# stcodeer/Frequency-wised_All-in-One_Image_Restoration_Model

Measured on AMD Instinct MI355X. Metric: training images/sec @128x128, higher is better.
Workload: dtype bf16; 1 GPU; BASELINE configs[1]: Uformer encoder+decoder (all_3_bands, L=3, freq MSA), denoise sigma=25, 128x128, phase-2 train step (fwd+bwd+Adam, DropPath on); per_gpu_batch=16, global_batch=16, parallelism=dp1, hip_graph=True

## Files before the change

### frequency-wised_all-in-one_image_restoration_model_amd/csrc/fw_gemm.hip

```cpp
#include "fw_common.h"
#include <stdio.h>
#include <string.h>
#include <stdlib.h>

namespace {
static thread_local char g_last_kernel[96] = "";
template <typename T> constexpr const char* tname() { return sizeof(T) == 2 ? "bf16" : "float"; }
#define FW_B(x) ((x) ? "true" : "false")
#define FW_KNAME(...) snprintf(g_last_kernel, sizeof g_last_kernel, __VA_ARGS__)

struct GemmArgs {
    const char* X; const char* W; char* C;
    long ldx, ldw, ldc;
    int M, N, K;
    int x_op, w_op;
    const float* bias;
    int act; float slope;
    const char* aux; long ldaux;
    const float* rowscale; int rows_per_scale;
    const float* residual; long ldr;
    int out_f32;
    int accumulate;
    int splitk; int kper;
    char* C2; long ldc2;
    float* xsum;
    long c_zstride, xsum_zstride;
    float alpha;
    int staged;
    int dbg;
};

constexpr int LDS_ROW = 128;
FW_DEV int swz(int row) { return ((row ^ (row >> 3)) & 7) << 4; }
constexpr int BM = 128;

FW_DEV unsigned xcd_contiguous(unsigned lin, unsigned total) {
    const unsigned xcd = lin & 7, q = total >> 3, r = total & 7;
    return (xcd < r ? xcd * (q + 1) : r * (q + 1) + (xcd - r) * q) + (lin >> 3);
}

template <typename T> FW_DEV uint4 apply_gelu16(const uint4& v) {
    float f[TT<T>::E16];
    unpack16<T>(v, f);
#pragma unroll
    for (int i = 0; i < TT<T>::E16; ++i) f[i] = gelu_t<T>(f[i]);
    return pack16<T>(f);
}

template <typename T>
FW_DEV void epi_fetch(const GemmArgs& a, uint4& ext, int mc, int nc, int z) {
    if (a.act == 2) {
        const T* ap = reinterpret_cast<const T*>(a.aux) + (long)mc * a.ldaux + nc;
        if (sizeof(T) == 4) ext = *reinterpret_cast<const uint4*>(ap);
        else { const uint2 t = *reinterpret_cast<const uint2*>(ap); ext.x = t.x; ext.y = t.y; }
    } else if (a.residual && z == 0) {
        ext = *reinterpret_cast<const uint4*>(a.residual + (long)mc * a.ldr + nc);
    }
}
FW_DEV f32x4 epi_bias(const GemmArgs& a, int nc, int z) {
    return (a.bias && z == 0) ? *reinterpret_cast<const f32x4*>(a.bias + nc) : f32x4{0.f, 0.f, 0.f, 0.f};
}
template <typename T>
FW_DEV void epi_apply(const GemmArgs& a, const f32x4& bias, const uint4& ext, const f32x4& acc, int m, int n0, float rs, int z) {
    float v[4];
#pragma unroll
    for (int r = 0; r < 4; ++r) v[r] = acc[r] * a.alpha + bias[r];
    if (a.act == 1) {
#pragma unroll
        for (int r = 0; r < 4; ++r) v[r] = lrelu_f(v[r], a.slope);
    } else if (a.act == 2) {
        float x[4];
        if (sizeof(T) == 4) { x[0] = __uint_as_float(ext.x); x[1] = __uint_as_float(ext.y); x[2] = __uint_as_float(ext.z); x[3] = __uint_as_float(ext.w); }
        else { x[0] = __uint_as_float(ext.x << 16); x[1] = __uint_as_float(ext.x & 0xffff0000u);
               x[2] = __uint_as_float(ext.y << 16); x[3] = __uint_as_float(ext.y & 0xffff0000u); }
#pragma unroll
        for (int r = 0; r < 4; ++r) v[r] *= gelu_grad_t<T>(x[r]);
    } else if (a.act == 3) {
#pragma unroll
        for (int r = 0; r < 4; ++r) v[r] = gelu_t<T>(v[r]);
    }
    if (a.rowscale) {
#pragma unroll
        for (int r = 0; r < 4; ++r) v[r] *= rs;
    }
    if (a.residual && z == 0) {
        uint4 rr = ext;
        if (a.act == 2) rr = *reinterpret_cast<const uint4*>(a.residual + (long)m * a.ldr + n0);
        v[0] += __uint_as_float(rr.x); v[1] += __uint_as_float(rr.y); v[2] += __uint_as_float(rr.z); v[3] += __uint_as_float(rr.w);
    }
    if (a.C2) {
        T* c2 = reinterpret_cast<T*>(a.C2) + (long)m * a.ldc2 + n0;
        const float g0 = gelu_t<T>(v[0]), g1 = gelu_t<T>(v[1]), g2 = gelu_t<T>(v[2]), g3 = gelu_t<T>(v[3]);
        if (sizeof(T) == 4) *reinterpret_cast<f32x4*>(c2) = f32x4{g0, g1, g2, g3};
        else *reinterpret_cast<uint2*>(c2) = make_uint2(pack_bf2(g0, g1), pack_bf2(g2, g3));
    }
    if (a.out_f32) {
        float* cp = reinterpret_cast<float*>(a.C) + (long)z * a.c_zstride + (long)m * a.ldc + n0;
        if (a.accumulate && a.c_zstride == 0) {
            if (a.accumulate == 1 && a.splitk == 1) {
                const f32x4 old = *reinterpret_cast<const f32x4*>(cp);
                *reinterpret_cast<f32x4*>(cp) = f32x4{old[0] + v[0], old[1] + v[1], old[2] + v[2], old[3] + v[3]};
            } else {
#pragma unroll
                for (int r = 0; r < 4; ++r) atomicAdd(cp + r, v[r]);
            }
        } else {
            *reinterpret_cast<f32x4*>(cp) = f32x4{v[0], v[1], v[2], v[3]};
        }
    } else {
        T* cp = reinterpret_cast<T*>(a.C) + (long)m * a.ldc + n0;
        if (sizeof(T) == 4) *reinterpret_cast<f32x4*>(cp) = f32x4{v[0], v[1], v[2], v[3]};
        else *reinterpret_cast<uint2*>(cp) = make_uint2(pack_bf2(v[0], v[1]), pack_bf2(v[2], v[3]));
    }
}

template <typename T, int ROWS>
struct StageDirect {
    static constexpr int NL = ROWS / 32;
    uint4 r[NL];
    FW_MEM void load(const char* base, long ld, int row0, int rows_total, int kbyte0, int kbytes_end, int op) {
        const int tid = threadIdx.x;
#pragma unroll
        for (int t = 0; t < NL; ++t) {
            const int cid = tid + 256 * t;
            const int row = cid >> 3, kb = kbyte0 + (cid & 7) * 16;
            const int rr = row0 + row < rows_total ? row0 + row : rows_total - 1;
            r[t] = *reinterpret_cast<const uint4*>(base + (long)rr * ld * TT<T>::SZ + (kb < kbytes_end ? kb : 0));
        }
#pragma unroll
        for (int t = 0; t < NL; ++t) {
            const int cid = tid + 256 * t;
            const int row = cid >> 3, kb = kbyte0 + (cid & 7) * 16;
            uint4 v = r[t];
            if (op == 1) v = apply_gelu16<T>(v);
            const int valid = row0 + row < rows_total ? kbytes_end - kb : 0;
            v.x = valid > 0 ? v.x : 0u; v.y = valid > 4 ? v.y : 0u; v.z = valid > 8 ? v.z : 0u; v.w = valid > 12 ? v.w : 0u;
            r[t] = v;
        }
    }
    FW_MEM void store(char* tile) const {
        const int tid = threadIdx.x;
#pragma unroll
        for (int t = 0; t < NL; ++t) {
            const int cid = tid + 256 * t;
            const int row = cid >> 3;
            *reinterpret_cast<uint4*>(tile + row * LDS_ROW + (((cid & 7) * 16) ^ swz(row))) = r[t];
        }
    }
};

template <typename T, int ROWS>
struct StageTrans {
    static constexpr int E = TT<T>::E16;
    static constexpr int IB = ROWS / E;
    static constexpr int KT = 128 / TT<T>::SZ;
    static constexpr int NTHR = IB * (KT / 4);
    uint4 r[4];
    FW_MEM void load(const char* base, long ld, int row0, int rows_total, int k0, int k_end, int op) {
        const int tid = threadIdx.x;
        const int ib = tid % IB, kb = tid / IB;
#pragma unroll
        for (int kk = 0; kk < 4; ++kk) {
            const int k = k0 + kb * 4 + kk;
            uint4 v = make_uint4(0, 0, 0, 0);
            if (tid < NTHR && k < k_end && row0 + ib * E < rows_total) {
                v = *reinterpret_cast<const uint4*>(base + ((long)k * ld + row0 + ib * E) * TT<T>::SZ);
                if (op == 1) v = apply_gelu16<T>(v);
            }
            r[kk] = v;
        }
    }
    FW_MEM void accum(float (&s)[TT<T>::E16]) const {
#pragma unroll
        for (int kk = 0; kk < 4; ++kk) {
            float f[TT<T>::E16];
            unpack16<T>(r[kk], f);
#pragma unroll
            for (int e = 0; e < TT<T>::E16; ++e) s[e] += f[e];
        }
    }
    FW_MEM void store(char* tile) const {
        const int tid = threadIdx.x;
        if (tid >= NTHR) return;
        const int ib = tid % IB, kb = tid / IB;
        if constexpr (sizeof(T) == 4) {
            const int r0 = ib * 4, cb = kb * 16;
            *reinterpret_cast<uint4*>(tile + (r0 + 0) * LDS_ROW + (cb ^ swz(r0 + 0))) = make_uint4(r[0].x, r[1].x, r[2].x, r[3].x);
            *reinterpret_cast<uint4*>(tile + (r0 + 1) * LDS_ROW + (cb ^ swz(r0 + 1))) = make_uint4(r[0].y, r[1].y, r[2].y, r[3].y);
            *reinterpret_cast<uint4*>(tile + (r0 + 2) * LDS_ROW + (cb ^ swz(r0 + 2))) = make_uint4(r[0].z, r[1].z, r[2].z, r[3].z);
            *reinterpret_cast<uint4*>(tile + (r0 + 3) * LDS_ROW + (cb ^ swz(r0 + 3))) = make_uint4(r[0].w, r[1].w, r[2].w, r[3].w);
        } else {
            const int r0 = ib * 8, cb = kb * 8;
            const unsigned w0[4] = {r[0].x, r[0].y, r[0].z, r[0].w};
            const unsigned w1[4] = {r[1].x, r[1].y, r[1].z, r[1].w};
            const unsigned w2[4] = {r[2].x, r[2].y, r[2].z, r[2].w};
            const unsigned w3[4] = {r[3].x, r[3].y, r[3].z, r[3].w};
#pragma unroll
            for (int d = 0; d < 4; ++d) {
                uint2 lo = make_uint2(__builtin_amdgcn_perm(w1[d], w0[d], 0x05040100u),
                                      __builtin_amdgcn_perm(w3[d], w2[d], 0x05040100u));
                uint2 hi = make_uint2(__builtin_amdgcn_perm(w1[d], w0[d], 0x07060302u),
                                      __builtin_amdgcn_perm(w3[d], w2[d], 0x07060302u));
                *reinterpret_cast<uint2*>(tile + (r0 + 2 * d) * LDS_ROW + (cb ^ swz(r0 + 2 * d))) = lo;
                *reinterpret_cast<uint2*>(tile + (r0 + 2 * d + 1) * LDS_ROW + (cb ^ swz(r0 + 2 * d + 1))) = hi;
            }
        }
    }
};

typedef __attribute__((address_space(3))) void lds_void_t;
typedef __attribute__((address_space(1))) const void glb_void_t;
template <typename T, int ROWS>
FW_DEV void glds_issue(const char* base, long ld, int row0, int rows_total, int kbyte0, char* tile) {
    const int lane = threadIdx.x & 63, wave = threadIdx.x >> 6;
#pragma unroll
    for (int it = 0; it < ROWS / 32; ++it) {
        const int R0 = (wave * (ROWS / 32) + it) * 8;
        const int r = R0 + (lane >> 3), p = lane & 7;
        int gr = row0 + r;
        if (gr >= rows_total) gr = rows_total - 1;
        const char* g = base + (long)gr * ld * TT<T>::SZ + kbyte0 + ((p ^ (swz(r) >> 4)) << 4);
        __builtin_amdgcn_global_load_lds((glb_void_t*)g, (lds_void_t*)(tile + R0 * LDS_ROW), 16, 0, 0);
    }
}

template <typename T, int ROWS> struct StageDirectAcc : StageDirect<T, ROWS> {
    FW_MEM void accum(float (&)[TT<T>::E16]) const {}
};
template <typename T, int ROWS, bool TRANS> struct Stage;
template <typename T, int ROWS> struct Stage<T, ROWS, false> : StageDirectAcc<T, ROWS> {
    FW_MEM void fetch(const char* base, long ld, int row0, int rows_total, int k0, int k_end, int op) {
        this->load(base, ld, row0, rows_total, k0 * TT<T>::SZ, k_end * TT<T>::SZ, op);
    }
};
template <typename T, int ROWS> struct Stage<T, ROWS, true> : StageTrans<T, ROWS> {
    FW_MEM void fetch(const char* base, long ld, int row0, int rows_total, int k0, int k_end, int op) {
        this->load(base, ld, row0, rows_total, k0, k_end, op);
    }
};

FW_DEV uint4 frag_sw(const char* tile, int row0, int chunk) {
    const int l = lane_id();
    const int row = row0 + (l & 15);
    return *reinterpret_cast<const uint4*>(tile + row * LDS_ROW + ((chunk * 64 + ((l >> 4) << 4)) ^ swz(row)));
}

template <typename T, int BN, bool XT, bool WT, bool GX, bool GW>
__global__ __launch_bounds__(256) void gemm_kernel(GemmArgs a) {
    constexpr int KT = 128 / TT<T>::SZ;
    constexpr int WM = (BN == 128) ? 4 : 2;
    constexpr int XBYTES = BM * LDS_ROW, WBYTES = BN * LDS_ROW;
    extern __shared__ __attribute__((aligned(16))) char smem[];
    auto xs = [&](int i) -> char* { return smem + i * (XBYTES + WBYTES); };
    auto ws = [&](int i) -> char* { return smem + i * (XBYTES + WBYTES) + XBYTES; };

    const int wave = threadIdx.x >> 6;
    int bx = blockIdx.x, by = blockIdx.y, bz = blockIdx.z;
    {
        const unsigned total = gridDim.x * gridDim.y * gridDim.z;
        if (gridDim.z > 1) {
            const unsigned lin = blockIdx.x + gridDim.x * (blockIdx.y + gridDim.y * blockIdx.z);
            const unsigned w = xcd_contiguous(lin, total);
            bx = (int)(w % gridDim.x);
            by = (int)((w / gridDim.x) % gridDim.y);
            bz = (int)(w / (gridDim.x * gridDim.y));
        } else if (gridDim.z == 1 && gridDim.y > 1) {
            const unsigned lin = blockIdx.x + gridDim.x * blockIdx.y;
            const unsigned w = xcd_contiguous(lin, total);
            const unsigned per_band = 8 * gridDim.y;
            const unsigned band = w / per_band, first = band * 8;
            const unsigned gsz = min(gridDim.x - first, 8u);
            bx = (int)(first + (w % per_band) % gsz);
            by = (int)((w % per_band) / gsz);
        }
    }
    const int m_blk = bx * BM, n_blk = by * BN;
    const int wm0 = (BN == 128) ? (wave & 1) * 64 : wave * 32;
    const int wn0 = (BN == 128) ? (wave >> 1) * 64 : 0;

    const int k_begin = bz * a.kper;
    const int k_end = min(a.K, k_begin + a.kper);
    const int nsteps = (k_end - k_begin + KT - 1) / KT;

    f32x4 acc[4][WM];
    zero_acc(acc);

    Stage<T, BM, XT> sx;
    Stage<T, BN, WT> sw;
    float xsum[TT<T>::E16];
#pragma unroll
    for (int e = 0; e < TT<T>::E16; ++e) xsum[e] = 0.f;
    const bool do_xsum = XT && a.xsum != nullptr && by == 0;
    if (nsteps > 0) {
        if constexpr (GX) glds_issue<T, BM>(a.X, a.ldx, m_blk, a.M, k_begin * TT<T>::SZ, xs(0));
        else { sx.fetch(a.X, a.ldx, m_blk, a.M, k_begin, k_end, a.x_op); if (do_xsum) sx.accum(xsum); }
        if constexpr (GW) glds_issue<T, BN>(a.W, a.ldw, n_blk, a.N, k_begin * TT<T>::SZ, ws(0));
        else sw.fetch(a.W, a.ldw, n_blk, a.N, k_begin, k_end, a.w_op);
        if constexpr (!GX) sx.store(xs(0));
        if constexpr (!GW) sw.store(ws(0));
    }
    __syncthreads();
    for (int s = 0; s < nsteps; ++s) {
        const int cur = s & 1;
        if (s + 1 < nsteps) {
            if constexpr (GX) glds_issue<T, BM>(a.X, a.ldx, m_blk, a.M, (k_begin + (s + 1) * KT) * TT<T>::SZ, xs(cur ^ 1));
            else { sx.fetch(a.X, a.ldx, m_blk, a.M, k_begin + (s + 1) * KT, k_end, a.x_op); if (do_xsum) sx.accum(xsum); }
            if constexpr (GW) glds_issue<T, BN>(a.W, a.ldw, n_blk, a.N, (k_begin + (s + 1) * KT) * TT<T>::SZ, ws(cur ^ 1));
            else sw.fetch(a.W, a.ldw, n_blk, a.N, k_begin + (s + 1) * KT, k_end, a.w_op);
        }
#pragma unroll
        for (int c = 0; c < 2; ++c) {
            uint4 af[4], bfr[WM];
#pragma unroll
            for (int m = 0; m < 4; ++m) af[m] = frag_sw(ws(cur), wn0 + 16 * m, c);
#pragma unroll
            for (int n = 0; n < WM; ++n) bfr[n] = frag_sw(xs(cur), wm0 + 16 * n, c);
#pragma unroll
            for (int m = 0; m < 4; ++m)
#pragma unroll
                for (int n = 0; n < WM; ++n) mma_chunk<T>(acc[m][n], af[m], bfr[n]);
        }
        if (s + 1 < nsteps) {
            if constexpr (!GX) sx.store(xs(cur ^ 1));
            if constexpr (!GW) sw.store(ws(cur ^ 1));
        }
        __syncthreads();
    }

    if constexpr (XT) {
        if (a.xsum != nullptr && by == 0) {
            constexpr int E = TT<T>::E16, IB = BM / E;
            float* red = reinterpret_cast<float*>(smem);
            if (threadIdx.x < BM) red[threadIdx.x] = 0.f;
            __syncthreads();
            if ((int)threadIdx.x < IB * ((128 / TT<T>::SZ) / 4)) {
                const int ib = threadIdx.x % IB;
#pragma unroll
                for (int e = 0; e < E; ++e) atomicAdd(&red[ib * E + e], xsum[e]);
            }
            __syncthreads();
            if (threadIdx.x < BM && m_blk + (int)threadIdx.x < a.M) {
                if (a.xsum_zstride > 0) a.xsum[(long)bz * a.xsum_zstride + m_blk + threadIdx.x] = red[threadIdx.x];
                else atomicAdd(a.xsum + m_blk + threadIdx.x, red[threadIdx.x]);
            }
        }
    }
    const int l = lane_id();
    f32x4 bias4[4];
#pragma unroll
    for (int nt = 0; nt < 4; ++nt) {
        const int n0 = n_blk + wn0 + nt * 16 + ((l >> 4) << 2);
        bias4[nt] = epi_bias(a, n0 < a.N ? n0 : 0, bz);
    }
#pragma unroll
    for (int mt = 0; mt < WM; ++mt) {
        const int m = m_blk + wm0 + mt * 16 + (l & 15);
        const int mc = m < a.M ? m : a.M - 1;
        const float rs = a.rowscale ? a.rowscale[mc / a.rows_per_scale] : 1.0f;
        uint4 ext[4];
#pragma unroll
        for (int nt = 0; nt < 4; ++nt) {
            const int n0 = n_blk + wn0 + nt * 16 + ((l >> 4) << 2);
            epi_fetch<T>(a, ext[nt], mc, n0 < a.N ? n0 : 0, bz);
        }
#pragma unroll
        for (int nt = 0; nt < 4; ++nt) {
            const int n0 = n_blk + wn0 + nt * 16 + ((l >> 4) << 2);
            if (m < a.M && n0 < a.N) epi_apply<T>(a, bias4[nt], ext[nt], acc[nt][mt], m, n0, rs, bz);
        }
    }
}

FW_DEV int swz256(int r) { return ((r & 3) << 2) | ((r >> 2) & 3); }

FW_DEV uint4 frag_tr256(const char* tile, int m0, int chunk) {
    const int l = lane_id();
    const int r = chunk * 32 + ((l >> 4) << 3) + ((l >> 2) & 3);
    const int ch = (m0 >> 3) + ((l & 3) >> 1), sub = (l & 1) << 3;
    const char* p0 = tile + 256 * r + ((ch ^ swz256(r)) << 4) + sub;
    const char* p1 = tile + 256 * (r + 4) + ((ch ^ swz256(r + 4)) << 4) + sub;
    const uint2 lo = __builtin_bit_cast(uint2, __builtin_amdgcn_ds_read_tr16_b64_v4i16((fw_lds_s16x4*)p0));
    const uint2 hi = __builtin_bit_cast(uint2, __builtin_amdgcn_ds_read_tr16_b64_v4i16((fw_lds_s16x4*)p1));
    return make_uint4(lo.x, lo.y, hi.x, hi.y);
}

template <typename T, int WM, bool PLAIN>
FW_DEV void tile_epilogue(const GemmArgs& a, const f32x4 (&acc)[4][WM], int m_blk, int n_blk, int wm0, int wn0, int bz) {
    const int l = lane_id();
    f32x4 bias4[4];
#pragma unroll
    for (int nt = 0; nt < 4; ++nt) {
        const int n0 = n_blk + wn0 + nt * 16 + ((l >> 4) << 2);
        bias4[nt] = epi_bias(a, n0 < a.N ? n0 : 0, bz);
    }
    if constexpr (PLAIN) {
#pragma unroll
        for (int mt = 0; mt < WM; ++mt) {
            const int m = m_blk + wm0 + mt * 16 + (l & 15);
            if (m >= a.M) continue;
            if (a.out_f32) {
                float* cp = reinterpret_cast<float*>(a.C) + (long)bz * a.c_zstride + (long)m * a.ldc;
#pragma unroll
                for (int nt = 0; nt < 4; ++nt) {
                    const int n0 = n_blk + wn0 + nt * 16 + ((l >> 4) << 2);
                    if (n0 < a.N) *reinterpret_cast<f32x4*>(cp + n0) = acc[nt][mt] + bias4[nt];
                }
            } else {
                T* cp = reinterpret_cast<T*>(a.C) + (long)m * a.ldc;
#pragma unroll
                for (int nt = 0; nt < 4; ++nt) {
                    const int n0 = n_blk + wn0 + nt * 16 + ((l >> 4) << 2);
                    if (n0 < a.N) {
                        const f32x4 v = acc[nt][mt] + bias4[nt];
                        if (sizeof(T) == 4) *reinterpret_cast<f32x4*>(cp + n0) = v;
                        else *reinterpret_cast<uint2*>(cp + n0) = make_uint2(pack_bf2(v[0], v[1]), pack_bf2(v[2], v[3]));
                    }
                }
            }
        }
    } else {
        const bool tw = sizeof(T) == 2 && a.alpha == 1.0f && !a.out_f32 && !a.rowscale && !a.residual && !a.accumulate;
        if (tw && a.act == 2 && !a.C2) {
            auto fetchA = [&](uint2 (&ext)[4], int mt) {
                const int m = m_blk + wm0 + mt * 16 + (l & 15);
                const T* ap = reinterpret_cast<const T*>(a.aux) + (long)(m < a.M ? m : a.M - 1) * a.ldaux;
#pragma unroll
                for (int nt = 0; nt < 4; ++nt) {
                    const int n0 = n_blk + wn0 + nt * 16 + ((l >> 4) << 2);
                    ext[nt] = *reinterpret_cast<const uint2*>(ap + (n0 < a.N ? n0 : 0));
                }
            };
            auto applyA = [&](const uint2 (&ext)[4], int mt) {
                const int m = m_blk + wm0 + mt * 16 + (l & 15);
                if (m >= a.M) return;
                T* cp = reinterpret_cast<T*>(a.C) + (long)m * a.ldc;
#pragma unroll
                for (int nt = 0; nt < 4; ++nt) {
                    const int n0 = n_blk + wn0 + nt * 16 + ((l >> 4) << 2);
                    if (n0 >= a.N) continue;
                    const f32x4 v = acc[nt][mt] + bias4[nt];
                    const float x0 = __uint_as_float(ext[nt].x << 16), x1 = __uint_as_float(ext[nt].x & 0xffff0000u);
                    const float x2 = __uint_as_float(ext[nt].y << 16), x3 = __uint_as_float(ext[nt].y & 0xffff0000u);
                    *reinterpret_cast<uint2*>(cp + n0) = make_uint2(pack_bf2(v[0] * gelu_grad_poly(x0), v[1] * gelu_grad_poly(x1)),
                                                                    pack_bf2(v[2] * gelu_grad_poly(x2), v[3] * gelu_grad_poly(x3)));
                }
            };
            uint2 ea[4], eb[4];
            fetchA(ea, 0);
#pragma unroll
            for (int mt = 0; mt < WM; mt += 2) {
                if (mt + 1 < WM) fetchA(eb, mt + 1);
                applyA(ea, mt);
                if (mt + 1 < WM) {
                    if (mt + 2 < WM) fetchA(ea, mt + 2);
                    applyA(eb, mt + 1);
                }
            }
            return;
        }
        if (tw && a.act == 0 && a.C2) {
#pragma unroll
            for (int mt = 0; mt < WM; ++mt) {
                const int m = m_blk + wm0 + mt * 16 + (l & 15);
                if (m >= a.M) continue;
                T* cp = reinterpret_cast<T*>(a.C) + (long)m * a.ldc;
                T* c2 = reinterpret_cast<T*>(a.C2) + (long)m * a.ldc2;
#pragma unroll
                for (int nt = 0; nt < 4; ++nt) {
                    const int n0 = n_blk + wn0 + nt * 16 + ((l >> 4) << 2);
                    if (n0 >= a.N) continue;
                    const f32x4 v = acc[nt][mt] + bias4[nt];
                    *reinterpret_cast<uint2*>(cp + n0) = make_uint2(pack_bf2(v[0], v[1]), pack_bf2(v[2], v[3]));
                    *reinterpret_cast<uint2*>(c2 + n0) = make_uint2(pack_bf2(gelu_poly(v[0]), gelu_poly(v[1])), pack_bf2(gelu_poly(v[2]), gelu_poly(v[3])));
                }
            }
            return;
        }
        if (a.act == 0 && a.residual && a.out_f32 && !a.C2 && a.alpha == 1.0f && !a.accumulate && a.splitk == 1 && a.c_zstride == 0) {
            auto fetchC = [&](f32x4 (&ext)[4], int mt) {
                const int m = m_blk + wm0 + mt * 16 + (l & 15);
                const float* rp = a.residual + (long)(m < a.M ? m : a.M - 1) * a.ldr;
#pragma unroll
                for (int nt = 0; nt < 4; ++nt) {
                    const int n0 = n_blk + wn0 + nt * 16 + ((l >> 4) << 2);
                    ext[nt] = *reinterpret_cast<const f32x4*>(rp + (n0 < a.N ? n0 : 0));
                }
            };
            auto applyC = [&](const f32x4 (&ext)[4], int mt) {
                const int m = m_blk + wm0 + mt * 16 + (l & 15);
                if (m >= a.M) return;
                const float rs = a.rowscale ? a.rowscale[m / a.rows_per_scale] : 1.0f;
                float* cp = reinterpret_cast<float*>(a.C) + (long)m * a.ldc;
#pragma unroll
                for (int nt = 0; nt < 4; ++nt) {
                    const int n0 = n_blk + wn0 + nt * 16 + ((l >> 4) << 2);
                    if (n0 < a.N) *reinterpret_cast<f32x4*>(cp + n0) = (acc[nt][mt] + bias4[nt]) * rs + ext[nt];
                }
            };
            f32x4 ea[4], eb[4];
            fetchC(ea, 0);
#pragma unroll
            for (int mt = 0; mt < WM; mt += 2) {
                if (mt + 1 < WM) fetchC(eb, mt + 1);
                applyC(ea, mt);
                if (mt + 1 < WM) {
                    if (mt + 2 < WM) fetchC(ea, mt + 2);
                    applyC(eb, mt + 1);
                }
            }
            return;
        }
        auto fetch = [&](uint4 (&ext)[4], int mt) {
            const int m = m_blk + wm0 + mt * 16 + (l & 15);
            const int mc = m < a.M ? m : a.M - 1;
#pragma unroll
            for (int nt = 0; nt < 4; ++nt) {
                const int n0 = n_blk + wn0 + nt * 16 + ((l >> 4) << 2);
                epi_fetch<T>(a, ext[nt], mc, n0 < a.N ? n0 : 0, bz);
            }
        };
        auto apply = [&](const uint4 (&ext)[4], int mt) {
            const int m = m_blk + wm0 + mt * 16 + (l & 15);
            const int mc = m < a.M ? m : a.M - 1;
            const float rs = a.rowscale ? a.rowscale[mc / a.rows_per_scale] : 1.0f;
#pragma unroll
            for (int nt = 0; nt < 4; ++nt) {
                const int n0 = n_blk + wn0 + nt * 16 + ((l >> 4) << 2);
                if (m < a.M && n0 < a.N) epi_apply<T>(a, bias4[nt], ext[nt], acc[nt][mt], m, n0, rs, bz);
            }
        };
        uint4 ea[4], eb[4];
        fetch(ea, 0);
#pragma unroll
        for (int mt = 0; mt < WM; mt += 2) {
            if (mt + 1 < WM) fetch(eb, mt + 1);
            apply(ea, mt);
            if (mt + 1 < WM) {
                if (mt + 2 < WM) fetch(ea, mt + 2);
                apply(eb, mt + 1);
            }
        }
    }
}
static inline bool plain_epilogue(const GemmArgs& a) {
    return a.act == 0 && !a.rowscale && !a.residual && !a.C2 && a.alpha == 1.0f && !(a.accumulate && a.c_zstride == 0);
}

template <int N> FW_DEV void wait_vmcnt() { asm volatile("s_waitcnt vmcnt(%0)" ::"n"(N) : "memory"); }
FW_DEV void glds16_asm(const char* gsrc, char* lds_dst) {
    unsigned keep;
    const unsigned dst = __builtin_amdgcn_readfirstlane((unsigned)(uintptr_t)(lds_void_t*)lds_dst);
    asm volatile("s_mov_b32 %0, m0\n\ts_mov_b32 m0, %2\n\ts_nop 0\n\tglobal_load_lds_dwordx4 %1, off\n\ts_mov_b32 m0, %0"
                 : "=&s"(keep) : "v"(gsrc), "s"(dst) : "memory");
}

template <int KT> struct GldsKm {
    static constexpr int NI = KT / 16;
    const char* src[NI];
    long kstride;
    int loff[NI];
    FW_MEM void init(const char* base, long ld, int col0, int cols_total, int k0) {
        const int lane = threadIdx.x & 63, wave = threadIdx.x >> 6;
        kstride = ld * 2;
#pragma unroll
        for (int it = 0; it < NI; ++it) {
            const int R0 = wave * (KT / 4) + it * 4;
            const int r = R0 + (lane >> 4), p = lane & 15;
            int col = col0 + ((p ^ swz256(r)) << 3);
            if (col >= cols_total) col = 0;
            src[it] = base + ((long)(k0 + r) * ld + col) * 2;
            loff[it] = R0 * 256;
        }
    }
    FW_MEM void issue(int step, char* tile) const {
        const long off = (long)step * KT * kstride;
#pragma unroll
        for (int it = 0; it < NI; ++it) glds16_asm(src[it] + off, tile + loff[it]);
    }
};
template <typename T, int ROWS> struct GldsKc {
    static constexpr int NI = ROWS / 32;
    const char* src[NI];
    int loff[NI];
    FW_MEM void init(const char* base, long ld, int row0, int rows_total, int kbyte0) {
        const int lane = threadIdx.x & 63, wave = threadIdx.x >> 6;
#pragma unroll
        for (int it = 0; it < NI; ++it) {
            const int R0 = (wave * NI + it) * 8;
            const int r = R0 + (lane >> 3), p = lane & 7;
            int gr = row0 + r;
            if (gr >= rows_total) gr = rows_total - 1;
            src[it] = base + (long)gr * ld * TT<T>::SZ + kbyte0 + ((p ^ (swz(r) >> 4)) << 4);
            loff[it] = R0 * LDS_ROW;
        }
    }
    FW_MEM void issue(int step, char* tile) const {
#pragma unroll
        for (int it = 0; it < NI; ++it) glds16_asm(src[it] + (long)step * 128, tile + loff[it]);
    }
};

constexpr int ROW64 = 64;
FW_DEV int swz64(int r) { return (r >> 2) & 3; }
template <typename T, int ROWS> struct GldsKc64 {
    static constexpr int NI = ROWS / 64;
    const char* src[NI];
    int loff[NI];
    FW_MEM void init(const char* base, long ld, int row0, int rows_total, int kbyte0) {
        const int lane = threadIdx.x & 63, wave = threadIdx.x >> 6;
#pragma unroll
        for (int it = 0; it < NI; ++it) {
            const int R0 = (wave * NI + it) * 16;
            const int r = R0 + (lane >> 2), p = lane & 3;
            int gr = row0 + r;
            if (gr >= rows_total) gr = rows_total - 1;
            src[it] = base + (long)gr * ld * TT<T>::SZ + kbyte0 + ((p ^ swz64(r)) << 4);
            loff[it] = R0 * ROW64;
        }
    }
    FW_MEM void issue(int step, char* tile) const {
#pragma unroll
        for (int it = 0; it < NI; ++it) glds16_asm(src[it] + (long)step * ROW64, tile + loff[it]);
    }
};
FW_DEV uint4 frag_sw64(const char* tile, int row0) {
    const int l = lane_id();
    const int row = row0 + (l & 15);
    return *reinterpret_cast<const uint4*>(tile + row * ROW64 + (((l >> 4) ^ swz64(row)) << 4));
}

constexpr int EPI_LD = 136;
template <int WM>
FW_DEV void tile_epilogue_staged(const GemmArgs& a, const f32x4 (&acc)[4][WM], int m_blk, int n_blk, int wm0, int wn0, char* stage, int mode) {
    const int l = lane_id();
    char* mine = stage + (threadIdx.x >> 6) * (16 * WM * EPI_LD);
    f32x4 bias4[4];
#pragma unroll
    for (int nt = 0; nt < 4; ++nt) {
        const int n0 = n_blk + wn0 + nt * 16 + ((l >> 4) << 2);
        bias4[nt] = epi_bias(a, n0 < a.N ? n0 : 0, 0);
    }
    const int rsub = l >> 3, cb = (l & 7) * 16;
    const int ncol = n_blk + wn0 + (l & 7) * 8;
    const bool col_ok = ncol < a.N;
    auto rows_out = [&](char* C, long ldc) {
#pragma unroll
        for (int it = 0; it < 2 * WM; ++it) {
            const int r = it * 8 + rsub, m = m_blk + wm0 + r;
            const uint4 v = *reinterpret_cast<const uint4*>(mine + r * EPI_LD + cb);
            if (m < a.M && col_ok) *reinterpret_cast<uint4*>(C + ((long)m * ldc + ncol) * 2) = v;
        }
    };
    if (mode == 2) {
#pragma unroll
        for (int it = 0; it < 2 * WM; ++it) {
            const int r = it * 8 + rsub, m = m_blk + wm0 + r;
            const long mc = m < a.M ? m : a.M - 1;
            const uint4 v = *reinterpret_cast<const uint4*>(a.aux + (mc * a.ldaux + (col_ok ? ncol : 0)) * 2);
            *reinterpret_cast<uint4*>(mine + r * EPI_LD + cb) = v;
        }
        __builtin_amdgcn_fence(__ATOMIC_RELEASE, "wavefront");
        asm volatile("s_waitcnt vmcnt(0) lgkmcnt(0)" ::: "memory");
        __builtin_amdgcn_fence(__ATOMIC_ACQUIRE, "wavefront");
    }
#pragma unroll
    for (int pass = 0; pass < 2; ++pass) {
        if (pass == 1 && mode != 1) break;
#pragma unroll
        for (int mt = 0; mt < WM; ++mt) {
            char* rowp = mine + (mt * 16 + (l & 15)) * EPI_LD + ((l >> 4) << 3);
#pragma unroll
            for (int nt = 0; nt < 4; ++nt) {
                f32x4 v = acc[nt][mt] + bias4[nt];
                if (mode == 2) {
                    const uint2 e = *reinterpret_cast<const uint2*>(rowp + nt * 32);
                    v[0] *= gelu_grad_poly(__uint_as_float(e.x << 16)); v[1] *= gelu_grad_poly(__uint_as_float(e.x & 0xffff0000u));
                    v[2] *= gelu_grad_poly(__uint_as_float(e.y << 16)); v[3] *= gelu_grad_poly(__uint_as_float(e.y & 0xffff0000u));
                } else if (pass == 1) {
                    v[0] = gelu_poly(v[0]); v[1] = gelu_poly(v[1]); v[2] = gelu_poly(v[2]); v[3] = gelu_poly(v[3]);
                }
                *reinterpret_cast<uint2*>(rowp + nt * 32) = make_uint2(pack_bf2(v[0], v[1]), pack_bf2(v[2], v[3]));
            }
        }
        __builtin_amdgcn_fence(__ATOMIC_RELEASE, "wavefront");
        asm volatile("s_waitcnt lgkmcnt(0)" ::: "memory");
        __builtin_amdgcn_fence(__ATOMIC_ACQUIRE, "wavefront");
        if (pass == 0) rows_out(a.C, a.ldc); else rows_out(a.C2, a.ldc2);
        if (pass == 0 && mode == 1) {
            __builtin_amdgcn_fence(__ATOMIC_RELEASE, "wavefront");
            asm volatile("s_waitcnt lgkmcnt(0)" ::: "memory");
            __builtin_amdgcn_fence(__ATOMIC_ACQUIRE, "wavefront");
        }
    }
}
static inline int staged_mode(const GemmArgs& a) {
    if (a.out_f32 || a.alpha != 1.0f || a.rowscale || a.residual || a.accumulate || a.c_zstride || a.splitk != 1 || a.N % 8 || a.ldc % 8) return -1;
    if (((uintptr_t)a.C & 15)) return -1;
    if (a.act == 0 && !a.C2) return 0;
    if (a.act == 0 && a.C2) return (a.ldc2 % 8 || ((uintptr_t)a.C2 & 15)) ? -1 : 1;
    if (a.act == 2 && !a.C2) return (a.ldaux % 8 || ((uintptr_t)a.aux & 15)) ? -1 : 2;
    return -1;
}

template <bool XT, int KT, int NS, bool PLAIN>
FW_DEV void tr_ring_tile(const GemmArgs& a, int bx, int by, int bz, char* smem) {
    using T = bf16raw;
    static_assert(NS == 2 || NS == 3, "ring depth");
    constexpr int WM = 4;
    constexpr bool X64 = !XT && KT == 32;
    constexpr int XB = XT ? KT * 256 : 128 * (X64 ? ROW64 : LDS_ROW), WB = KT * 256, STAGE = XB + WB;
    constexpr int LPS = (XT ? KT / 16 : (X64 ? 2 : 4)) + KT / 16;
    auto xs = [&](int i) -> char* { return smem + i * STAGE; };
    auto ws = [&](int i) -> char* { return smem + i * STAGE + XB; };
    const int wave = threadIdx.x >> 6;
    const int m_blk = bx * 128, n_blk = by * 128;
    const int wm0 = (wave & 1) * 64, wn0 = (wave >> 1) * 64;
    const int k_begin = bz * a.kper;
    const int k_end = min(a.K, k_begin + a.kper);
    const int nsteps = (k_end - k_begin) / KT;

    f32x4 acc[4][WM], xsacc[WM];
    zero_acc(acc);
#pragma unroll
    for (int m = 0; m < WM; ++m) xsacc[m] = f32x4{0.f, 0.f, 0.f, 0.f};
    const bool do_xsum = XT && a.xsum != nullptr && by == 0 && wn0 == 0;
    const uint4 ones = make_uint4(0x3F803F80u, 0x3F803F80u, 0x3F803F80u, 0x3F803F80u);

    GldsKm<KT> gw;
    gw.init(a.W, a.ldw, n_blk, a.N, k_begin);
    GldsKm<XT ? KT : 16> gxm;
    GldsKc<T, BM> gxc;
    GldsKc64<T, BM> gxc64;
    if constexpr (XT) gxm.init(a.X, a.ldx, m_blk, a.M, k_begin);
    else if constexpr (X64) gxc64.init(a.X, a.ldx, m_blk, a.M, k_begin * 2);
    else gxc.init(a.X, a.ldx, m_blk, a.M, k_begin * 2);
    auto issue = [&](int step, int buf) {
        if constexpr (XT) gxm.issue(step, xs(buf));
        else if constexpr (X64) gxc64.issue(step, xs(buf));
        else gxc.issue(step, xs(buf));
        gw.issue(step, ws(buf));
    };
#pragma unroll
    for (int p = 0; p < NS - 1; ++p)
        if (p < nsteps) issue(p, p);
    int buf = 0;
    for (int s = 0; s < nsteps; ++s) {
        const int younger = min(NS - 2, nsteps - 1 - s);
        if (younger >= NS - 2) wait_vmcnt<(NS - 2) * LPS>();
        else wait_vmcnt<0>();
        __builtin_amdgcn_s_barrier();
        asm volatile("" ::: "memory");
        if (s + NS - 1 < nsteps) issue(s + NS - 1, buf == 0 ? NS - 1 : buf - 1);
#pragma unroll
        for (int c = 0; c < KT / 32; ++c) {
            uint4 af[4], bfr[WM];
#pragma unroll
            for (int m = 0; m < 4; ++m) af[m] = frag_tr256(ws(buf), wn0 + 16 * m, c);
#pragma unroll
            for (int n = 0; n < WM; ++n) bfr[n] = XT ? frag_tr256(xs(buf), wm0 + 16 * n, c) : (X64 ? frag_sw64(xs(buf), wm0 + 16 * n) : frag_sw(xs(buf), wm0 + 16 * n, c));
#pragma unroll
            for (int m = 0; m < 4; ++m)
#pragma unroll
                for (int n = 0; n < WM; ++n) mma_chunk<T>(acc[m][n], af[m], bfr[n]);
            if (do_xsum) {
#pragma unroll
                for (int n = 0; n < WM; ++n) mma_chunk<T>(xsacc[n], ones, bfr[n]);
            }
        }
        buf = buf + 1 == NS ? 0 : buf + 1;
    }
    const int l = lane_id();
    if (do_xsum && (l >> 4) == 0) {
#pragma unroll
        for (int n = 0; n < WM; ++n) {
            const int m = m_blk + wm0 + n * 16 + l;
            if (m < a.M) {
                if (a.xsum_zstride > 0) a.xsum[(long)bz * a.xsum_zstride + m] = xsacc[n][0];
                else atomicAdd(a.xsum + m, xsacc[n][0]);
            }
        }
    }
    if (a.staged >= 0 && (size_t)NS * STAGE >= (size_t)4 * 16 * WM * EPI_LD) {
        __syncthreads();
        tile_epilogue_staged<WM>(a, acc, m_blk, n_blk, wm0, wn0, smem, a.staged);
        return;
    }
    tile_epilogue<T, WM, PLAIN>(a, acc, m_blk, n_blk, wm0, wn0, bz);
}

template <bool XT, int KT, int NS, bool PLAIN>
__global__ __launch_bounds__(256, KT == 32 ? 3 : 2) void gemm_tr_ring_kernel(GemmArgs a) {
    extern __shared__ __attribute__((aligned(16))) char smem[];
    int bx = blockIdx.x, by = blockIdx.y, bz = blockIdx.z;
    {
        const unsigned total = gridDim.x * gridDim.y * gridDim.z;
        if (gridDim.z > 1) {
            const unsigned lin = blockIdx.x + gridDim.x * (blockIdx.y + gridDim.y * blockIdx.z);
            const unsigned w = xcd_contiguous(lin, total);
            bx = (int)(w % gridDim.x);
            by = (int)((w / gridDim.x) % gridDim.y);
            bz = (int)(w / (gridDim.x * gridDim.y));
        } else if (gridDim.z == 1 && gridDim.y > 1) {
            const unsigned lin = blockIdx.x + gridDim.x * blockIdx.y;
            const unsigned w = xcd_contiguous(lin, total);
            const unsigned per_band = 8 * gridDim.y;
            const unsigned band = w / per_band, first = band * 8;
            const unsigned gsz = min(gridDim.x - first, 8u);
            bx = (int)(first + (w % per_band) % gsz);
            by = (int)((w % per_band) / gsz);
        }
    }
    tr_ring_tile<XT, KT, NS, PLAIN>(a, bx, by, bz, smem);
}

__global__ __launch_bounds__(256, 3) void gemm_wgrad_group_kernel(const GemmArgs* __restrict__ probs, const int4* __restrict__ items) {
    extern __shared__ __attribute__((aligned(16))) char smem[];
    const int4 it = items[blockIdx.x];
    if (it.x < 0) return;
    const GemmArgs a = probs[it.x];
    if (a.c_zstride > 0) tr_ring_tile<true, 32, 3, true>(a, it.y, it.z, it.w, smem);
    else tr_ring_tile<true, 32, 3, false>(a, it.y, it.z, it.w, smem);
}

template <bool PLAIN>
FW_DEV void tr_big_tile(const GemmArgs& a, int bx, int by, int bz, char* smem) {
    using T = bf16raw;
    constexpr int KT = 32, NS = 3, WM = 8, IMG = KT * 256, STAGE = 4 * IMG, LPS = 4;
    const int lane = threadIdx.x & 63, wave = threadIdx.x >> 6;
    const int m_blk = bx * 256, n_blk = by * 256;
    const int wm0 = (wave & 1) * 128, wn0 = (wave >> 1) * 64;
    const int k_begin = bz * a.kper;
    const int k_end = min(a.K, k_begin + a.kper);
    const int nsteps = (k_end - k_begin) / KT;
    const char* src[4]; int off[4];
    {
        const bool isw = wave >= 4;
        const int half = (wave >> 1) & 1, rg = wave & 1;
        const char* base = isw ? a.W : a.X;
        const long ld = isw ? a.ldw : a.ldx;
        const int col0 = (isw ? n_blk : m_blk) + half * 128, cols = isw ? a.N : a.M;
#pragma unroll
        for (int it = 0; it < 4; ++it) {
            const int R0 = rg * 16 + it * 4, r = R0 + (lane >> 4), p = lane & 15;
            int col = col0 + ((p ^ swz256(r)) << 3);
            if (col >= cols) col = 0;
            src[it] = base + ((long)(k_begin + r) * ld + col) * 2;
            off[it] = (isw ? 2 * IMG : 0) + half * IMG + R0 * 256;
        }
    }
    const long kstride = (wave >= 4 ? a.ldw : a.ldx) * 2;
    auto issue = [&](int step, int buf) {
        char* st = smem + buf * STAGE;
#pragma unroll
        for (int it = 0; it < 4; ++it) glds16_asm(src[it] + (long)step * KT * kstride, st + off[it]);
    };
    f32x4 acc[4][WM];
    zero_acc(acc);
    float xs[WM];
#pragma unroll
    for (int m = 0; m < WM; ++m) xs[m] = 0.f;
    const bool do_xsum = a.xsum != nullptr && by == 0 && wn0 == 0;
    typedef __attribute__((ext_vector_type(2))) __bf16 bf2_t;
    const bf2_t ones2 = __builtin_bit_cast(bf2_t, 0x3F803F80u);
#pragma unroll
    for (int p = 0; p < NS - 1; ++p)
        if (p < nsteps) issue(p, p);
    int buf = 0;
    for (int s = 0; s < nsteps; ++s) {
        const int younger = min(NS - 2, nsteps - 1 - s);
        if (younger >= NS - 2) wait_vmcnt<(NS - 2) * LPS>();
        else wait_vmcnt<0>();
        __builtin_amdgcn_s_barrier();
        asm volatile("" ::: "memory");
        if (s + NS - 1 < nsteps) issue(s + NS - 1, buf == 0 ? NS - 1 : buf - 1);
        const char* st = smem + buf * STAGE;
        uint4 af[4], bfr[WM];
#pragma unroll
        for (int m = 0; m < 4; ++m) af[m] = frag_tr256(st + 2 * IMG + (wn0 >> 7) * IMG, (wn0 & 127) + 16 * m, 0);
#pragma unroll
        for (int n = 0; n < WM; ++n) bfr[n] = frag_tr256(st + (wm0 >> 7) * IMG, 16 * n, 0);
#pragma unroll
        for (int m = 0; m < 4; ++m)
#pragma unroll
            for (int n = 0; n < WM; ++n) mma_chunk<T>(acc[m][n], af[m], bfr[n]);
        if (do_xsum) {
#pragma unroll
            for (int n = 0; n < WM; ++n) {
                xs[n] = __builtin_amdgcn_fdot2_f32_bf16(__builtin_bit_cast(bf2_t, bfr[n].x), ones2, xs[n], false);
                xs[n] = __builtin_amdgcn_fdot2_f32_bf16(__builtin_bit_cast(bf2_t, bfr[n].y), ones2, xs[n], false);
                xs[n] = __builtin_amdgcn_fdot2_f32_bf16(__builtin_bit_cast(bf2_t, bfr[n].z), ones2, xs[n], false);
                xs[n] = __builtin_amdgcn_fdot2_f32_bf16(__builtin_bit_cast(bf2_t, bfr[n].w), ones2, xs[n], false);
            }
        }
        buf = buf + 1 == NS ? 0 : buf + 1;
    }
    const int l = lane_id();
    if (do_xsum) {
#pragma unroll
        for (int n = 0; n < WM; ++n) {
            float v = xs[n];
            v += __shfl_xor(v, 16, 64); v += __shfl_xor(v, 32, 64);
            const int m = m_blk + wm0 + n * 16 + l;
            if ((l >> 4) == 0 && m < a.M) {
                if (a.xsum_zstride > 0) a.xsum[(long)bz * a.xsum_zstride + m] = v;
                else atomicAdd(a.xsum + m, v);
            }
        }
    }
    tile_epilogue<T, WM, PLAIN>(a, acc, m_blk, n_blk, wm0, wn0, bz);
}
__global__ __launch_bounds__(512) void gemm_wgrad_group_big_kernel(const GemmArgs* __restrict__ probs, const int4* __restrict__ items) {
    extern __shared__ __attribute__((aligned(16))) char smem[];
    const int4 it = items[blockIdx.x];
    if (it.x < 0) return;
    const GemmArgs a = probs[it.x];
    if (a.c_zstride > 0) tr_big_tile<true>(a, it.y, it.z, it.w, smem);
    else tr_big_tile<false>(a, it.y, it.z, it.w, smem);
}

template <bool XT, int KT, int NS, bool PLAIN>
int launch_tr_ring_p(const GemmArgs& a, hipStream_t st) {
    const size_t lds = (size_t)NS * ((XT ? KT * 256 : 128 * ((KT == 32) ? ROW64 : LDS_ROW)) + KT * 256);
    FW_SET_LDS_ONCE((gemm_tr_ring_kernel<XT, KT, NS, PLAIN>), lds);
    FW_KNAME("gemm_tr_ring_kernel<%s,%d,%d,%s>", FW_B(XT), KT, NS, FW_B(PLAIN));
    hipLaunchKernelGGL((gemm_tr_ring_kernel<XT, KT, NS, PLAIN>), dim3(fw_cdiv(a.M, 128), fw_cdiv(a.N, 128), a.splitk), dim3(256), lds, st, a);
    FW_LAUNCH_RET();
}
template <bool XT, int KT, int NS>
int launch_tr_ring(const GemmArgs& a, hipStream_t st) {
    return plain_epilogue(a) ? launch_tr_ring_p<XT, KT, NS, true>(a, st) : launch_tr_ring_p<XT, KT, NS, false>(a, st);
}

template <typename T, int BN, int NS, bool PLAIN>
__global__ __launch_bounds__(256) void gemm_ring_kernel(GemmArgs a) {
    constexpr int KT = 128 / TT<T>::SZ;
    constexpr int WM = (BN == 128) ? 4 : 2;
    constexpr int XBYTES = BM * LDS_ROW, WBYTES = BN * LDS_ROW, STAGE = XBYTES + WBYTES;
    constexpr int LPS = BM / 32 + BN / 32;
    extern __shared__ __attribute__((aligned(16))) char smem[];
    auto xs = [&](int i) -> char* { return smem + i * STAGE; };
    auto ws = [&](int i) -> char* { return smem + i * STAGE + XBYTES; };
    const int wave = threadIdx.x >> 6;
    int bx = blockIdx.x, by = blockIdx.y, bz = blockIdx.z;
    {
        const unsigned total = gridDim.x * gridDim.y * gridDim.z;
        if (gridDim.z > 1) {
            const unsigned lin = blockIdx.x + gridDim.x * (blockIdx.y + gridDim.y * blockIdx.z);
            const unsigned w = xcd_contiguous(lin, total);
            bx = (int)(w % gridDim.x);
            by = (int)((w / gridDim.x) % gridDim.y);
            bz = (int)(w / (gridDim.x * gridDim.y));
        } else if (gridDim.z == 1 && gridDim.y > 1) {
            const unsigned lin = blockIdx.x + gridDim.x * blockIdx.y;
            const unsigned w = xcd_contiguous(lin, total);
            const unsigned per_band = 8 * gridDim.y;
            const unsigned band = w / per_band, first = band * 8;
            const unsigned gsz = min(gridDim.x - first, 8u);
            bx = (int)(first + (w % per_band) % gsz);
            by = (int)((w % per_band) / gsz);
        }
    }
    const int m_blk = bx * BM, n_blk = by * BN;
    const int wm0 = (BN == 128) ? (wave & 1) * 64 : wave * 32;
    const int wn0 = (BN == 128) ? (wave >> 1) * 64 : 0;
    const int k_begin = bz * a.kper;
    const int k_end = min(a.K, k_begin + a.kper);
    const int nsteps = (k_end - k_begin) / KT;

    f32x4 acc[4][WM];
    zero_acc(acc);
    GldsKc<T, BM> gx;
    GldsKc<T, BN> gw;
    gx.init(a.X, a.ldx, m_blk, a.M, k_begin * TT<T>::SZ);
    gw.init(a.W, a.ldw, n_blk, a.N, k_begin * TT<T>::SZ);
    auto issue = [&](int step, int buf) {
        gx.issue(step, xs(buf));
        gw.issue(step, ws(buf));
    };
#pragma unroll
    for (int p = 0; p < NS - 1; ++p)
        if (p < nsteps) issue(p, p);
    int buf = 0;
    for (int s = 0; s < nsteps; ++s) {
        const int younger = min(NS - 2, nsteps - 1 - s);
        if (younger >= NS - 2) wait_vmcnt<(NS - 2) * LPS>();
        else wait_vmcnt<0>();
        __builtin_amdgcn_s_barrier();
        asm volatile("" ::: "memory");
        if (s + NS - 1 < nsteps) issue(s + NS - 1, buf == 0 ? NS - 1 : buf - 1);
#pragma unroll
        for (int c = 0; c < 2; ++c) {
            uint4 af[4], bfr[WM];
#pragma unroll
            for (int m = 0; m < 4; ++m) af[m] = frag_sw(ws(buf), wn0 + 16 * m, c);
#pragma unroll
            for (int n = 0; n < WM; ++n) bfr[n] = frag_sw(xs(buf), wm0 + 16 * n, c);
#pragma unroll
            for (int m = 0; m < 4; ++m)
#pragma unroll
                for (int n = 0; n < WM; ++n) mma_chunk<T>(acc[m][n], af[m], bfr[n]);
        }
        buf = buf + 1 == NS ? 0 : buf + 1;
    }
    if constexpr (sizeof(T) == 2) {
        if (a.staged >= 0 && (size_t)NS * STAGE >= (size_t)4 * 16 * WM * EPI_LD) {
            __syncthreads();
            tile_epilogue_staged<WM>(a, acc, m_blk, n_blk, wm0, wn0, smem, a.staged);
            return;
        }
    }
    tile_epilogue<T, WM, PLAIN>(a, acc, m_blk, n_blk, wm0, wn0, bz);
}

template <typename T, int BN, int NS, bool PLAIN>
int launch_ring_p(const GemmArgs& a, hipStream_t st) {
    const size_t lds = (size_t)NS * (BM + BN) * LDS_ROW;
    FW_SET_LDS_ONCE((gemm_ring_kernel<T, BN, NS, PLAIN>), lds);
    dim3 grid(fw_cdiv(a.M, BM), fw_cdiv(a.N, BN), a.splitk);
    FW_KNAME("gemm_ring_kernel<%s,%d,%d,%s>", tname<T>(), BN, NS, FW_B(PLAIN));
    hipLaunchKernelGGL((gemm_ring_kernel<T, BN, NS, PLAIN>), grid, dim3(256), lds, st, a);
    FW_LAUNCH_RET();
}
template <typename T, int BN, int NS>
int launch_ring(const GemmArgs& a, hipStream_t st) {
    return plain_epilogue(a) ? launch_ring_p<T, BN, NS, true>(a, st) : launch_ring_p<T, BN, NS, false>(a, st);
}

template <typename T, int BN, int NS, bool PLAIN>
__global__ __launch_bounds__(256) void gemm_ring64_kernel(GemmArgs a) {
    constexpr int KT = ROW64 / TT<T>::SZ;
    constexpr int WM = (BN == 128) ? 4 : 2;
    constexpr int XBYTES = BM * ROW64, WBYTES = BN * ROW64, STAGE = XBYTES + WBYTES;
    constexpr int LPS = BM / 64 + BN / 64;
    static_assert(NS >= 3, "ring depth");
    extern __shared__ __attribute__((aligned(16))) char smem[];
    auto xs = [&](int i) -> char* { return smem + i * STAGE; };
    auto ws = [&](int i) -> char* { return smem + i * STAGE + XBYTES; };
    const int wave = threadIdx.x >> 6;
    int bx = blockIdx.x, by = blockIdx.y, bz = blockIdx.z;
    {
        const unsigned total = gridDim.x * gridDim.y * gridDim.z;
        if (gridDim.z > 1) {
            const unsigned lin = blockIdx.x + gridDim.x * (blockIdx.y + gridDim.y * blockIdx.z);
            const unsigned w = xcd_contiguous(lin, total);
            bx = (int)(w % gridDim.x);
            by = (int)((w / gridDim.x) % gridDim.y);
            bz = (int)(w / (gridDim.x * gridDim.y));
        } else if (gridDim.z == 1 && gridDim.y > 1) {
            const unsigned lin = blockIdx.x + gridDim.x * blockIdx.y;
            const unsigned w = xcd_contiguous(lin, total);
            const unsigned per_band = 8 * gridDim.y;
            const unsigned band = w / per_band, first = band * 8;
            const unsigned gsz = min(gridDim.x - first, 8u);
            bx = (int)(first + (w % per_band) % gsz);
            by = (int)((w % per_band) / gsz);
        }
    }
    const int m_blk = bx * BM, n_blk = by * BN;
    const int wm0 = (BN == 128) ? (wave & 1) * 64 : wave * 32;
    const int wn0 = (BN == 128) ? (wave >> 1) * 64 : 0;
    const int k_begin = bz * a.kper;
    const int k_end = min(a.K, k_begin + a.kper);
    const int nsteps = (k_end - k_begin) / KT;

    f32x4 acc[4][WM];
    zero_acc(acc);
    GldsKc64<T, BM> gx;
    GldsKc64<T, BN> gw;
    gx.init(a.X, a.ldx, m_blk, a.M, k_begin * TT<T>::SZ);
    gw.init(a.W, a.ldw, n_blk, a.N, k_begin * TT<T>::SZ);
    auto issue = [&](int step, int buf) {
        gx.issue(step, xs(buf));
        gw.issue(step, ws(buf));
    };
#pragma unroll
    for (int p = 0; p < NS - 1; ++p)
        if (p < nsteps) issue(p, p);
    int buf = 0;
    for (int s = 0; s < nsteps; ++s) {
        const int younger = min(NS - 2, nsteps - 1 - s);
        if (younger >= NS - 2) wait_vmcnt<(NS - 2) * LPS>();
        else if (younger == NS - 3) wait_vmcnt<(NS - 3) * LPS>();
        else wait_vmcnt<0>();
        __builtin_amdgcn_s_barrier();
        asm volatile("" ::: "memory");
        if (s + NS - 1 < nsteps) issue(s + NS - 1, buf == 0 ? NS - 1 : buf - 1);
        uint4 af[4], bfr[WM];
#pragma unroll
        for (int m = 0; m < 4; ++m) af[m] = frag_sw64(ws(buf), wn0 + 16 * m);
#pragma unroll
        for (int n = 0; n < WM; ++n) bfr[n] = frag_sw64(xs(buf), wm0 + 16 * n);
#pragma unroll
        for (int m = 0; m < 4; ++m)
#pragma unroll
            for (int n = 0; n < WM; ++n) mma_chunk<T>(acc[m][n], af[m], bfr[n]);
        buf = buf + 1 == NS ? 0 : buf + 1;
    }
    if constexpr (sizeof(T) == 2) {
        if (a.staged >= 0 && (size_t)NS * STAGE >= (size_t)4 * 16 * WM * EPI_LD) {
            __syncthreads();
            tile_epilogue_staged<WM>(a, acc, m_blk, n_blk, wm0, wn0, smem, a.staged);
            return;
        }
    }
    tile_epilogue<T, WM, PLAIN>(a, acc, m_blk, n_blk, wm0, wn0, bz);
}

template <typename T, int BN, int NS, bool PLAIN>
int launch_ring64_p(const GemmArgs& a, hipStream_t st) {
    const size_t lds = (size_t)NS * (BM + BN) * ROW64;
    FW_SET_LDS_ONCE((gemm_ring64_kernel<T, BN, NS, PLAIN>), lds);
    dim3 grid(fw_cdiv(a.M, BM), fw_cdiv(a.N, BN), a.splitk);
    FW_KNAME("gemm_ring64_kernel<%s,%d,%d,%s>", tname<T>(), BN, NS, FW_B(PLAIN));
    hipLaunchKernelGGL((gemm_ring64_kernel<T, BN, NS, PLAIN>), grid, dim3(256), lds, st, a);
    FW_LAUNCH_RET();
}
template <typename T, int BN, int NS>
int launch_ring64(const GemmArgs& a, hipStream_t st) {
    return plain_epilogue(a) ? launch_ring64_p<T, BN, NS, true>(a, st) : launch_ring64_p<T, BN, NS, false>(a, st);
}

template <bool WT, bool PLAIN>
__global__ __launch_bounds__(512) void gemm_big_kernel(GemmArgs a) {
    using T = bf16raw;
    constexpr int KT = 64, NS = 2, WM = 8, BIG = 256;
    constexpr int XB = BIG * LDS_ROW, WB = WT ? 2 * KT * 256 : XB, STAGE = XB + WB;
    constexpr int NIX = 4, NIW = 4, LPS = NIX + NIW;
    extern __shared__ __attribute__((aligned(16))) char smem[];
    auto xs = [&](int i) -> char* { return smem + i * STAGE; };
    auto ws = [&](int i) -> char* { return smem + i * STAGE + XB; };
    const int lane = threadIdx.x & 63, wave = threadIdx.x >> 6;
    int bx = blockIdx.x, by = blockIdx.y;
    if (gridDim.y > 1) {
        const unsigned total = gridDim.x * gridDim.y;
        const unsigned lin = blockIdx.x + gridDim.x * blockIdx.y;
        const unsigned w = xcd_contiguous(lin, total);
        const unsigned per_band = 8 * gridDim.y;
        const unsigned band = w / per_band, first = band * 8;
        const unsigned gsz = min(gridDim.x - first, 8u);
        bx = (int)(first + (w % per_band) % gsz);
        by = (int)((w % per_band) / gsz);
    }
    const int m_blk = bx * BIG, n_blk = by * BIG;
    const int wm0 = (wave & 1) * 128, wn0 = (wave >> 1) * 64;
    const int nsteps = a.K / KT;

    const char* xsrc[NIX]; int xoff[NIX];
    const char* wsrc[NIW]; int woff[NIW];
    long wkstride = 0;
#pragma unroll
    for (int it = 0; it < NIX; ++it) {
        const int R0 = (wave * NIX + it) * 8, r = R0 + (lane >> 3), p = lane & 7;
        int gr = m_blk + r; if (gr >= a.M) gr = a.M - 1;
        xsrc[it] = a.X + (long)gr * a.ldx * 2 + ((p ^ (swz(r) >> 4)) << 4);
        xoff[it] = R0 * LDS_ROW;
    }
    if constexpr (!WT) {
#pragma unroll
        for (int it = 0; it < NIW; ++it) {
            const int R0 = (wave * NIW + it) * 8, r = R0 + (lane >> 3), p = lane & 7;
            int gr = n_blk + r; if (gr >= a.N) gr = a.N - 1;
            wsrc[it] = a.W + (long)gr * a.ldw * 2 + ((p ^ (swz(r) >> 4)) << 4);
            woff[it] = R0 * LDS_ROW;
        }
    } else {
        const int half = wave >> 2, wq = wave & 3;
        wkstride = a.ldw * 2;
#pragma unroll
        for (int it = 0; it < NIW; ++it) {
            const int R0 = wq * (KT / 4) + it * 4, r = R0 + (lane >> 4), p = lane & 15;
            int col = n_blk + half * 128 + ((p ^ swz256(r)) << 3);
            if (col >= a.N) col = 0;
            wsrc[it] = a.W + ((long)r * a.ldw + col) * 2;
            woff[it] = half * KT * 256 + R0 * 256;
        }
    }
    auto issue = [&](int step, int buf) {
        char* xt = xs(buf); char* wt = ws(buf);
#pragma unroll
        for (int it = 0; it < NIX; ++it) glds16_asm(xsrc[it] + (long)step * KT * 2, xt + xoff[it]);
#pragma unroll
        for (int it = 0; it < NIW; ++it) glds16_asm(wsrc[it] + (WT ? (long)step * KT * wkstride : (long)step * KT * 2), wt + woff[it]);
    };
    f32x4 acc[4][WM];
    zero_acc(acc);
    const bool noload = a.dbg & 2;
#pragma unroll
    for (int p = 0; p < NS - 1; ++p)
        if (p < nsteps && !noload) issue(p, p);
    int buf = 0;
    for (int s = 0; s < nsteps; ++s) {
        const int younger = min(NS - 2, nsteps - 1 - s);
        if (younger >= NS - 2) wait_vmcnt<(NS - 2) * LPS>();
        else wait_vmcnt<0>();
        __builtin_amdgcn_s_barrier();
        asm volatile("" ::: "memory");
        if (s + NS - 1 < nsteps && !noload) issue(s + NS - 1, buf == 0 ? NS - 1 : buf - 1);
        const char* xt = xs(buf); const char* wt = ws(buf);
#pragma unroll
        for (int c = 0; c < KT / 32; ++c) {
            uint4 af[4], bfr[WM];
#pragma unroll
            for (int m = 0; m < 4; ++m) {
                if constexpr (WT) af[m] = frag_tr256(wt + (wn0 >> 7) * KT * 256, (wn0 & 127) + 16 * m, c);
                else af[m] = frag_sw(wt, wn0 + 16 * m, c);
            }
#pragma unroll
            for (int n = 0; n < WM; ++n) bfr[n] = frag_sw(xt, wm0 + 16 * n, c);
#pragma unroll
            for (int m = 0; m < 4; ++m)
#pragma unroll
                for (int n = 0; n < WM; ++n) mma_chunk<T>(acc[m][n], af[m], bfr[n]);
        }
        buf = buf + 1 == NS ? 0 : buf + 1;
    }
    if ((a.dbg & 1) && acc[0][0][0] != 12345.678f) return;
    if (a.staged >= 0) {
        __syncthreads();
        tile_epilogue_staged<WM>(a, acc, m_blk, n_blk, wm0, wn0, smem, a.staged);
        return;
    }
    tile_epilogue<T, WM, PLAIN>(a, acc, m_blk, n_blk, wm0, wn0, 0);
}

template <bool WT, bool PLAIN>
__global__ __launch_bounds__(256, 2) void gemm_wide_kernel(GemmArgs a) {
    using T = bf16raw;
    constexpr int KT = 32, NS = 3, WM = 8, TM = 128, TN = 256;
    constexpr int XB = TM * ROW64, WB = WT ? 2 * KT * 256 : TN * ROW64, STAGE = XB + WB;
    constexpr int NIX = 2, NIW = 4, LPS = NIX + NIW;
    extern __shared__ __attribute__((aligned(16))) char smem[];
    auto xs = [&](int i) -> char* { return smem + i * STAGE; };
    auto ws = [&](int i) -> char* { return smem + i * STAGE + XB; };
    const int lane = threadIdx.x & 63, wave = threadIdx.x >> 6;
    int bx = blockIdx.x, by = blockIdx.y;
    if (gridDim.y > 1) {
        const unsigned total = gridDim.x * gridDim.y;
        const unsigned lin = blockIdx.x + gridDim.x * blockIdx.y;
        const unsigned w = xcd_contiguous(lin, total);
        const unsigned per_band = 8 * gridDim.y;
        const unsigned band = w / per_band, first = band * 8;
        const unsigned gsz = min(gridDim.x - first, 8u);
        bx = (int)(first + (w % per_band) % gsz);
        by = (int)((w % per_band) / gsz);
    }
    const int m_blk = bx * TM, n_blk = by * TN;
    const int wm0 = 0, wn0 = wave * 64;
    const int nsteps = a.K / KT;
    const char* xsrc[NIX]; int xoff[NIX];
    const char* wsrc[NIW]; int woff[NIW];
    long wkstride = 0;
#pragma unroll
    for (int it = 0; it < NIX; ++it) {
        const int R0 = (wave * NIX + it) * 16, r = R0 + (lane >> 2), p = lane & 3;
        int gr = m_blk + r; if (gr >= a.M) gr = a.M - 1;
        xsrc[it] = a.X + (long)gr * a.ldx * 2 + ((p ^ swz64(r)) << 4);
        xoff[it] = R0 * ROW64;
    }
    if constexpr (!WT) {
#pragma unroll
        for (int it = 0; it < NIW; ++it) {
            const int R0 = (wave * NIW + it) * 16, r = R0 + (lane >> 2), p = lane & 3;
            int gr = n_blk + r; if (gr >= a.N) gr = a.N - 1;
            wsrc[it] = a.W + (long)gr * a.ldw * 2 + ((p ^ swz64(r)) << 4);
            woff[it] = R0 * ROW64;
        }
    } else {
        const int half = wave >> 1, wq = wave & 1;
        wkstride = a.ldw * 2;
#pragma unroll
        for (int it = 0; it < NIW; ++it) {
            const int R0 = wq * 16 + it * 4, r = R0 + (lane >> 4), p = lane & 15;
            int col = n_blk + half * 128 + ((p ^ swz256(r)) << 3);
            if (col >= a.N) col = 0;
            wsrc[it] = a.W + ((long)r * a.ldw + col) * 2;
            woff[it] = half * KT * 256 + R0 * 256;
        }
    }
    auto issue = [&](int step, int buf) {
        char* xt = xs(buf); char* wt = ws(buf);
#pragma unroll
        for (int it = 0; it < NIX; ++it) glds16_asm(xsrc[it] + (long)step * KT * 2, xt + xoff[it]);
#pragma unroll
        for (int it = 0; it < NIW; ++it) glds16_asm(wsrc[it] + (WT ? (long)step * KT * wkstride : (long)step * KT * 2), wt + woff[it]);
    };
    f32x4 acc[4][WM];
    zero_acc(acc);
#pragma unroll
    for (int p = 0; p < NS - 1; ++p)
        if (p < nsteps) issue(p, p);
    int buf = 0;
    for (int s = 0; s < nsteps; ++s) {
        const int younger = min(NS - 2, nsteps - 1 - s);
        if (younger >= NS - 2) wait_vmcnt<(NS - 2) * LPS>();
        else wait_vmcnt<0>();
        __builtin_amdgcn_s_barrier();
        asm volatile("" ::: "memory");
        if (s + NS - 1 < nsteps) issue(s + NS - 1, buf == 0 ? NS - 1 : buf - 1);
        const char* xt = xs(buf); const char* wt = ws(buf);
        uint4 af[4], bfr[WM];
#pragma unroll
        for (int m = 0; m < 4; ++m) {
            if constexpr (WT) af[m] = frag_tr256(wt + (wn0 >> 7) * KT * 256, (wn0 & 127) + 16 * m, 0);
            else af[m] = frag_sw64(wt, wn0 + 16 * m);
        }
#pragma unroll
        for (int n = 0; n < WM; ++n) bfr[n] = frag_sw64(xt, wm0 + 16 * n);
#pragma unroll
        for (int m = 0; m < 4; ++m)
#pragma unroll
            for (int n = 0; n < WM; ++n) mma_chunk<T>(acc[m][n], af[m], bfr[n]);
        buf = buf + 1 == NS ? 0 : buf + 1;
    }
    if (a.staged >= 0) {
        __syncthreads();
        tile_epilogue_staged<WM>(a, acc, m_blk, n_blk, wm0, wn0, smem, a.staged);
        return;
    }
    tile_epilogue<T, WM, PLAIN>(a, acc, m_blk, n_blk, wm0, wn0, 0);
}
template <bool WT, bool PLAIN>
int launch_wide_p(const GemmArgs& a, hipStream_t st) {
    size_t lds = (size_t)3 * (128 * ROW64 + (WT ? 2 * 32 * 256 : 256 * ROW64));
    if (lds < (size_t)4 * 128 * EPI_LD) lds = (size_t)4 * 128 * EPI_LD;
    FW_SET_LDS_ONCE((gemm_wide_kernel<WT, PLAIN>), lds);
    FW_KNAME("gemm_wide_kernel<%s,%s>", FW_B(WT), FW_B(PLAIN));
    hipLaunchKernelGGL((gemm_wide_kernel<WT, PLAIN>), dim3(fw_cdiv(a.M, 128), fw_cdiv(a.N, 256), 1), dim3(256), lds, st, a);
    FW_LAUNCH_RET();
}

template <bool WT, bool PLAIN>
int launch_big_p(const GemmArgs& a, hipStream_t st) {
    size_t lds = (size_t)2 * (256 * LDS_ROW + (WT ? 2 * 64 * 256 : 256 * LDS_ROW));
    if (lds < (size_t)8 * 128 * EPI_LD) lds = (size_t)8 * 128 * EPI_LD;
    FW_SET_LDS_ONCE((gemm_big_kernel<WT, PLAIN>), lds);
    FW_KNAME("gemm_big_kernel<%s,%s>", FW_B(WT), FW_B(PLAIN));
    hipLaunchKernelGGL((gemm_big_kernel<WT, PLAIN>), dim3(fw_cdiv(a.M, 256), fw_cdiv(a.N, 256), 1), dim3(512), lds, st, a);
    FW_LAUNCH_RET();
}
template <bool WT>
int launch_big(const GemmArgs& a, hipStream_t st) {
    constexpr int BIG_MIN_N = 16384;
    const bool pl = plain_epilogue(a);
    if (a.N >= BIG_MIN_N) return pl ? launch_big_p<WT, true>(a, st) : launch_big_p<WT, false>(a, st);
    return pl ? launch_wide_p<WT, true>(a, st) : launch_wide_p<WT, false>(a, st);
}

#define STREAM_HOT(NCH, EXT) (!((NCH) == 8 && (EXT) != 0))
#define STREAM_MTS(NCH, EXT) 2

template <int NCH, int EXT, int NB>
FW_DEV int stream_hot_strips(const GemmArgs& a, char* smem, const int bnp, const int n_blk, int strip, const int stride, const int full) {
    using T = bf16raw;
    constexpr int MTS = 2, RL = NCH * 64, ROWS = 16 * MTS;
    constexpr int ESZ = EXT == 2 ? 4 : 2;
    static_assert(STREAM_MTS(NCH, EXT) == MTS, "strip height");
    const int l = lane_id(), wave = __builtin_amdgcn_readfirstlane(threadIdx.x >> 6);
    strip = __builtin_amdgcn_readfirstlane(strip);
    const int kbytes = a.K * 2;
    const float* sbias = reinterpret_cast<const float*>(smem + (size_t)bnp * RL);
    struct XSet { uint4 v[MTS][NCH]; };
    struct ESet { uint4 v[MTS][4]; float rs[MTS]; };
    const int ncols = min(bnp, a.N - n_blk);
    unsigned xoff[NCH];
#pragma unroll
    for (int c = 0; c < NCH; ++c) {
        const int kb = c * 64 + ((l >> 4) << 4);
        xoff[c] = (unsigned)(l & 15) * (unsigned)a.ldx * 2u + (unsigned)(kb < kbytes ? kb : 0);
    }
    auto issue_x = [&](XSet& x, int s) {
#pragma unroll
        for (int mt = 0; mt < MTS; ++mt) {
            const char* src = a.X + (long)(s * ROWS + mt * 16) * a.ldx * 2;
#pragma unroll
            for (int c = 0; c < NCH; ++c) x.v[mt][c] = *reinterpret_cast<const uint4*>(src + xoff[c]);
        }
    };
    auto mask_x = [&](XSet& x) {
#pragma unroll
        for (int mt = 0; mt < MTS; ++mt) {
#pragma unroll
            for (int c = 0; c < NCH; ++c) {
                const int valid = kbytes - (c * 64 + ((l >> 4) << 4));
                uint4 v = x.v[mt][c];
                v.x = valid > 0 ? v.x : 0u; v.y = valid > 4 ? v.y : 0u; v.z = valid > 8 ? v.z : 0u; v.w = valid > 12 ? v.w : 0u;
                x.v[mt][c] = v;
            }
        }
    };
    const long lde = EXT == 1 ? a.ldaux : a.ldr;
    const char* ebase = EXT == 1 ? a.aux : reinterpret_cast<const char*>(a.residual);
    auto quad_ok = [&](int j, int i, int l) { return j < NB - 1 || j * 64 + i * 16 + ((l >> 4) << 2) < ncols; };
    auto fetch_e = [&](ESet& e, int s, int j) {
#pragma unroll
        for (int mt = 0; mt < MTS; ++mt) {
            const char* src = ebase + ((long)(s * ROWS + mt * 16) * lde + n_blk + j * 64) * ESZ;
#pragma unroll
            for (int i = 0; i < 4; ++i) {
                const unsigned off = ((unsigned)(l & 15) * (unsigned)lde + (quad_ok(j, i, l) ? (unsigned)(i * 16 + ((l >> 4) << 2)) : 0u)) * ESZ;
                if constexpr (EXT == 1) {
                    const uint2 t = *reinterpret_cast<const uint2*>(src + off);
                    e.v[mt][i].x = t.x; e.v[mt][i].y = t.y;
                } else {
                    e.v[mt][i] = *reinterpret_cast<const uint4*>(src + off);
                }
            }
        }
    };
    const bool has_rs = a.rowscale != nullptr;
    const float* rsp = has_rs ? a.rowscale : a.residual;
    const unsigned rs_div = has_rs ? (unsigned)max(a.rows_per_scale, 1) : 0x80000000u;
    auto fetch_rs = [&](ESet& e, int s) {
#pragma unroll
        for (int mt = 0; mt < MTS; ++mt) e.rs[mt] = rsp[(unsigned)(s * ROWS + mt * 16 + (l & 15)) / rs_div];
    };
    auto pin_x = [&](XSet& x) {
#pragma unroll
        for (int mt = 0; mt < MTS; ++mt) {
#pragma unroll
            for (int c = 0; c < NCH; ++c) asm volatile("" : "+v"(x.v[mt][c].x), "+v"(x.v[mt][c].y), "+v"(x.v[mt][c].z), "+v"(x.v[mt][c].w) : : "memory");
        }
    };
    auto pin_e = [&](ESet& e) {
#pragma unroll
        for (int mt = 0; mt < MTS; ++mt) {
#pragma unroll
            for (int i = 0; i < 4; ++i) {
                if constexpr (EXT == 1) asm volatile("" : "+v"(e.v[mt][i].x), "+v"(e.v[mt][i].y) : : "memory");
                else asm volatile("" : "+v"(e.v[mt][i].x), "+v"(e.v[mt][i].y), "+v"(e.v[mt][i].z), "+v"(e.v[mt][i].w) : : "memory");
            }
            if constexpr (EXT == 2) asm volatile("" : "+v"(e.rs[mt]) : : "memory");
        }
    };
    auto block_mma = [&](f32x4 (&acc)[4][MTS], const XSet& x, int j, int l) {
        zero_acc(acc);
#pragma unroll
        for (int c = 0; c < NCH; ++c) {
            uint4 af[4];
#pragma unroll
            for (int i = 0; i < 4; ++i) {
                const int row = j * 64 + i * 16 + (l & 15);
                af[i] = *reinterpret_cast<const uint4*>(smem + row * RL + ((c * 64 + ((l >> 4) << 4)) ^ swz(row)));
            }
#pragma unroll
            for (int i = 0; i < 4; ++i) {
#pragma unroll
                for (int mt = 0; mt < MTS; ++mt) mma_chunk<T>(acc[i][mt], af[i], x.v[mt][c]);
            }
        }
    };
    auto block_out = [&](const f32x4 (&acc)[4][MTS], const ESet& e, int s, int j, int l) {
        if constexpr (EXT == 0) {
            char* mine = smem + (size_t)bnp * RL + (size_t)bnp * 4 + wave * (16 * EPI_LD);
            const int chunk = j == NB - 1 ? min(l & 7, ((ncols - j * 64) >> 3) - 1) : (l & 7);
            const int rsub = l >> 3, cb = chunk * 16;
            const unsigned coff = ((unsigned)rsub * (unsigned)a.ldc + (unsigned)chunk * 8u) * 2u;
#pragma unroll
            for (int mt = 0; mt < MTS; ++mt) {
                char* rowp = mine + (l & 15) * EPI_LD + ((l >> 4) << 3);
#pragma unroll
                for (int i = 0; i < 4; ++i) {
                    const f32x4 v = acc[i][mt] + *reinterpret_cast<const f32x4*>(sbias + j * 64 + i * 16 + ((l >> 4) << 2));
                    *reinterpret_cast<uint2*>(rowp + i * 32) = make_uint2(pack_bf2(v[0], v[1]), pack_bf2(v[2], v[3]));
                }
                __builtin_amdgcn_fence(__ATOMIC_RELEASE, "wavefront");
                asm volatile("s_waitcnt lgkmcnt(0)" ::: "memory");
                __builtin_amdgcn_fence(__ATOMIC_ACQUIRE, "wavefront");
#pragma unroll
                for (int it = 0; it < 2; ++it) {
                    const uint4 v = *reinterpret_cast<const uint4*>(mine + (it * 8 + rsub) * EPI_LD + cb);
                    char* cp = a.C + ((long)(s * ROWS + mt * 16 + it * 8) * a.ldc + n_blk + j * 64) * 2;
                    *reinterpret_cast<uint4*>(cp + coff) = v;
                }
                __builtin_amdgcn_fence(__ATOMIC_RELEASE, "wavefront");
                asm volatile("s_waitcnt lgkmcnt(0)" ::: "memory");
                __builtin_amdgcn_fence(__ATOMIC_ACQUIRE, "wavefront");
            }
        } else {
#pragma unroll
            for (int mt = 0; mt < MTS; ++mt) {
                char* cp = a.C + ((long)(s * ROWS + mt * 16) * a.ldc + n_blk + j * 64) * ESZ;
                unsigned coff0 = 0;
                uint2 pk0 = make_uint2(0u, 0u);
                float v0[4] = {0.f, 0.f, 0.f, 0.f};
#pragma unroll
                for (int i = 0; i < 4; ++i) {
                    const int nq = j * 64 + i * 16 + ((l >> 4) << 2);
                    unsigned coff = ((unsigned)(l & 15) * (unsigned)a.ldc + (unsigned)(i * 16 + ((l >> 4) << 2))) * ESZ;
                    const bool ok = j < NB - 1 || i == 0 || quad_ok(j, i, l);
                    const f32x4 b = *reinterpret_cast<const f32x4*>(sbias + nq);
                    const uint4 ex = e.v[mt][i];
                    float v[4];
#pragma unroll
                    for (int r = 0; r < 4; ++r) v[r] = acc[i][mt][r] + b[r];
                    if constexpr (EXT == 1) {
                        v[0] *= gelu_grad_t<T>(__uint_as_float(ex.x << 16)); v[1] *= gelu_grad_t<T>(__uint_as_float(ex.x & 0xffff0000u));
                        v[2] *= gelu_grad_t<T>(__uint_as_float(ex.y << 16)); v[3] *= gelu_grad_t<T>(__uint_as_float(ex.y & 0xffff0000u));
                        uint2 pk = make_uint2(pack_bf2(v[0], v[1]), pack_bf2(v[2], v[3]));
                        if (i == 0) { pk0 = pk; coff0 = coff; }
                        pk.x = ok ? pk.x : pk0.x; pk.y = ok ? pk.y : pk0.y; coff = ok ? coff : coff0;
                        *reinterpret_cast<uint2*>(cp + coff) = pk;
                    } else {
                        const float rr[4] = {__uint_as_float(ex.x), __uint_as_float(ex.y), __uint_as_float(ex.z), __uint_as_float(ex.w)};
#pragma unroll
                        for (int r = 0; r < 4; ++r) v[r] = __fadd_rn(__fmul_rn(v[r], has_rs ? e.rs[mt] : 1.0f), rr[r]);
                        if (i == 0) { coff0 = coff; v0[0] = v[0]; v0[1] = v[1]; v0[2] = v[2]; v0[3] = v[3]; }
#pragma unroll
                        for (int r = 0; r < 4; ++r) v[r] = ok ? v[r] : v0[r];
                        coff = ok ? coff : coff0;
                        *reinterpret_cast<f32x4*>(cp + coff) = f32x4{v[0], v[1], v[2], v[3]};
                    }
                }
            }
        }
    };
    XSet xc, xn;
    ESet ec, en;
    issue_x(xc, strip);
    if constexpr (EXT != 0) fetch_e(ec, strip, 0);
    if constexpr (EXT == 2) fetch_rs(ec, strip);
    mask_x(xc);
    if constexpr (EXT != 0) pin_e(ec);
    auto strip_blocks = [&](int s) {
        asm volatile("" ::: "memory");
#pragma unroll
        for (int j = 0; j < NB; ++j) {
            f32x4 acc[4][MTS];
            int lj = l;
            asm volatile("" : "+v"(lj));
            block_mma(acc, xc, j, lj);
            ESet ea;
            if constexpr (EXT != 0) { if (j + 1 < NB) fetch_e(ea, s, j + 1); }
            if constexpr (EXT == 2) { ea.rs[0] = ec.rs[0]; ea.rs[1] = ec.rs[1]; }
            block_out(acc, ec, s, j, lj);
            if constexpr (EXT != 0) { if (j + 1 < NB) ec = ea; }
        }
    };
#pragma unroll 1
    for (; strip + stride < full; strip += stride) {
        issue_x(xn, strip + stride);
        if constexpr (EXT != 0) fetch_e(en, strip + stride, 0);
        if constexpr (EXT == 2) fetch_rs(en, strip + stride);
        strip_blocks(strip);
        __builtin_amdgcn_sched_barrier(0);
        pin_x(xn);
        xc = xn;
        mask_x(xc);
        if constexpr (EXT != 0) { ec = en; pin_e(ec); }
    }
    strip_blocks(strip);
    return strip + stride;
}

template <typename T, int NCH, bool WT, int EXT>
__global__ __launch_bounds__(512, (NCH == 2 && !EXT) ? 4 : 2) void gemm_stream_kernel(GemmArgs a, int bnp, int hot) {
    constexpr int SZ = TT<T>::SZ, E = TT<T>::E16;
    constexpr int RL = NCH * 64;
    constexpr int MTS = STREAM_MTS(NCH, EXT);
    extern __shared__ __attribute__((aligned(16))) char smem[];
    int l = lane_id();
    const int wave = threadIdx.x >> 6;
    const int n_blk = blockIdx.y * bnp;
    const int kbytes = a.K * SZ;

    if constexpr (!WT) {
        constexpr int SLOTS = RL / 16;
        for (int idx = threadIdx.x; idx < bnp * SLOTS; idx += 512) {
            const int row = idx / SLOTS, kb = (idx % SLOTS) * 16;
            uint4 v = make_uint4(0, 0, 0, 0);
            if (n_blk + row < a.N && kb < kbytes) {
                v = *reinterpret_cast<const uint4*>(a.W + (long)(n_blk + row) * a.ldw * SZ + kb);
                const int valid = kbytes - kb;
                if (valid < 16) {
                    if (valid <= 12) v.w = 0;
                    if (valid <= 8) v.z = 0;
                    if (valid <= 4) v.y = 0;
                }
            }
            *reinterpret_cast<uint4*>(smem + row * RL + (kb ^ swz(row))) = v;
        }
    } else {
        constexpr int KQ = RL / (4 * SZ);
        const int nblocks = bnp / E;
        for (int idx = threadIdx.x; idx < KQ * nblocks; idx += 512) {
            const int ib = idx % nblocks, kq = idx / nblocks;
            uint4 r[4];
#pragma unroll
            for (int kk = 0; kk < 4; ++kk) {
                const int k = kq * 4 + kk;
                r[kk] = make_uint4(0, 0, 0, 0);
                if (k < a.K && n_blk + ib * E < a.N) r[kk] = *reinterpret_cast<const uint4*>(a.W + ((long)k * a.ldw + n_blk + ib * E) * SZ);
            }
            if constexpr (sizeof(T) == 4) {
                const int r0 = ib * 4, cb = kq * 16;
                *reinterpret_cast<uint4*>(smem + (r0 + 0) * RL + (cb ^ swz(r0 + 0))) = make_uint4(r[0].x, r[1].x, r[2].x, r[3].x);
                *reinterpret_cast<uint4*>(smem + (r0 + 1) * RL + (cb ^ swz(r0 + 1))) = make_uint4(r[0].y, r[1].y, r[2].y, r[3].y);
                *reinterpret_cast<uint4*>(smem + (r0 + 2) * RL + (cb ^ swz(r0 + 2))) = make_uint4(r[0].z, r[1].z, r[2].z, r[3].z);
                *reinterpret_cast<uint4*>(smem + (r0 + 3) * RL + (cb ^ swz(r0 + 3))) = make_uint4(r[0].w, r[1].w, r[2].w, r[3].w);
            } else {
                const int r0 = ib * 8, cb = kq * 8;
                const unsigned w0[4] = {r[0].x, r[0].y, r[0].z, r[0].w};
                const unsigned w1[4] = {r[1].x, r[1].y, r[1].z, r[1].w};
                const unsigned w2[4] = {r[2].x, r[2].y, r[2].z, r[2].w};
                const unsigned w3[4] = {r[3].x, r[3].y, r[3].z, r[3].w};
#pragma unroll
                for (int d = 0; d < 4; ++d) {
                    const uint2 lo = make_uint2(__builtin_amdgcn_perm(w1[d], w0[d], 0x05040100u), __builtin_amdgcn_perm(w3[d], w2[d], 0x05040100u));
                    const uint2 hi = make_uint2(__builtin_amdgcn_perm(w1[d], w0[d], 0x07060302u), __builtin_amdgcn_perm(w3[d], w2[d], 0x07060302u));
                    *reinterpret_cast<uint2*>(smem + (r0 + 2 * d) * RL + (cb ^ swz(r0 + 2 * d))) = lo;
                    *reinterpret_cast<uint2*>(smem + (r0 + 2 * d + 1) * RL + (cb ^ swz(r0 + 2 * d + 1))) = hi;
                }
            }
        }
    }
    {
        float* sb = reinterpret_cast<float*>(smem + (size_t)bnp * RL);
        for (int i = threadIdx.x; i < bnp; i += 512) sb[i] = (a.bias && n_blk + i < a.N) ? a.bias[n_blk + i] : 0.f;
    }
    __syncthreads();

    const int strips = (a.M + 16 * MTS - 1) / (16 * MTS);
    const int stride = gridDim.x * 8;
    const int ncols = min(bnp, a.N - n_blk);
    const int nnb = (ncols + 63) >> 6;
    uint4 xf[MTS][NCH];
    auto issue_x = [&](int strip) {
#pragma unroll
        for (int mt = 0; mt < MTS; ++mt) {
            const int row = strip * (16 * MTS) + mt * 16 + (l & 15);
            const char* src = a.X + (long)(row < a.M ? row : a.M - 1) * a.ldx * SZ;
#pragma unroll
            for (int c = 0; c < NCH; ++c) {
                const int kb = c * 64 + ((l >> 4) << 4);
                xf[mt][c] = *reinterpret_cast<const uint4*>(src + (kb < kbytes ? kb : 0));
            }
        }
    };
    auto mask_x = [&](int strip) {
#pragma unroll
        for (int mt = 0; mt < MTS; ++mt) {
            const bool rok = strip * (16 * MTS) + mt * 16 + (l & 15) < a.M;
#pragma unroll
            for (int c = 0; c < NCH; ++c) {
                const int valid = rok ? kbytes - (c * 64 + ((l >> 4) << 4)) : 0;
                uint4 v = xf[mt][c];
                v.x = valid > 0 ? v.x : 0u; v.y = valid > 4 ? v.y : 0u; v.z = valid > 8 ? v.z : 0u; v.w = valid > 12 ? v.w : 0u;
                xf[mt][c] = v;
            }
        }
    };
    const float* sbias = reinterpret_cast<const float*>(smem + (size_t)bnp * RL);
    int strip = blockIdx.x * 8 + wave;
    if constexpr (sizeof(T) == 2 && STREAM_HOT(NCH, EXT)) {
        const int full = a.M / (16 * MTS);
        if (hot && strip < full) {
            switch (nnb) {
            case 1: strip = stream_hot_strips<NCH, EXT, 1>(a, smem, bnp, n_blk, strip, stride, full); break;
            case 2: strip = stream_hot_strips<NCH, EXT, 2>(a, smem, bnp, n_blk, strip, stride, full); break;
            case 3: strip = stream_hot_strips<NCH, EXT, 3>(a, smem, bnp, n_blk, strip, stride, full); break;
            case 4: strip = stream_hot_strips<NCH, EXT, 4>(a, smem, bnp, n_blk, strip, stride, full); break;
            default: break;
            }
        }
        asm volatile("" : "+v"(l));
    }
    if (strip < strips) issue_x(strip);
    for (; strip < strips; strip += stride) {
        asm volatile("" : "+v"(l));
        mask_x(strip);
        const int m_lane = strip * (16 * MTS) + (l & 15);
        float rs[MTS];
#pragma unroll
        for (int mt = 0; mt < MTS; ++mt) {
            const int m = m_lane + mt * 16;
            rs[mt] = a.rowscale ? a.rowscale[(m < a.M ? m : a.M - 1) / a.rows_per_scale] : 1.0f;
        }
        if constexpr (EXT == 1 && NCH <= 4 && sizeof(T) == 4) {
            constexpr int EW = sizeof(T) == 2 ? 1 : 2;
            struct ExtSet { uint2 v[MTS][4][EW]; };
            auto fetch_ext = [&](ExtSet& e, int nb) {
#pragma unroll
                for (int mt = 0; mt < MTS; ++mt) {
                    const int m = m_lane + mt * 16;
                    const T* ap = reinterpret_cast<const T*>(a.aux) + (long)(m < a.M ? m : a.M - 1) * a.ldaux;
#pragma unroll
                    for (int i = 0; i < 4; ++i) {
                        const int n0 = n_blk + nb * 64 + i * 16 + ((l >> 4) << 2);
                        const uint2* src = reinterpret_cast<const uint2*>(ap + (n0 < a.N ? n0 : 0));
#pragma unroll
                        for (int q = 0; q < EW; ++q) e.v[mt][i][q] = src[q];
                    }
                }
            };
            auto block = [&](int nb, const ExtSet& cur, ExtSet& nxt) {
                f32x4 acc[4][MTS];
                zero_acc(acc);
#pragma unroll
                for (int c = 0; c < NCH; ++c) {
                    uint4 af[4];
#pragma unroll
                    for (int i = 0; i < 4; ++i) {
                        const int row = nb * 64 + i * 16 + (l & 15);
                        af[i] = *reinterpret_cast<const uint4*>(smem + row * RL + ((c * 64 + ((l >> 4) << 4)) ^ swz(row)));
                    }
#pragma unroll
                    for (int i = 0; i < 4; ++i) {
#pragma unroll
                        for (int mt = 0; mt < MTS; ++mt) mma_chunk<T>(acc[i][mt], af[i], xf[mt][c]);
                    }
                }
                if (nb + 1 < nnb) fetch_ext(nxt, nb + 1);
                if (nb == nnb - 1 && strip + stride < strips) issue_x(strip + stride);
#pragma unroll
                for (int mt = 0; mt < MTS; ++mt) {
                    const int m = m_lane + mt * 16;
#pragma unroll
                    for (int i = 0; i < 4; ++i) {
                        const int n0 = n_blk + nb * 64 + i * 16 + ((l >> 4) << 2);
                        const uint4 ex = EW == 1 ? make_uint4(cur.v[mt][i][0].x, cur.v[mt][i][0].y, 0u, 0u)
                                                 : make_uint4(cur.v[mt][i][0].x, cur.v[mt][i][0].y, cur.v[mt][i][EW - 1].x, cur.v[mt][i][EW - 1].y);
                        if (m < a.M && n0 < a.N) epi_apply<T>(a, *reinterpret_cast<const f32x4*>(sbias + (n0 - n_blk)), ex, acc[i][mt], m, n0, rs[mt], 0);
                    }
                }
            };
            ExtSet ea, eb;
            fetch_ext(ea, 0);
#pragma unroll 1
            for (int nb = 0; nb < nnb; nb += 2) {
                block(nb, ea, eb);
                if (nb + 1 < nnb) block(nb + 1, eb, ea);
            }
        } else {
#pragma unroll 1
            for (int nb = 0; nb < nnb; ++nb) {
                f32x4 acc[4][MTS];
                zero_acc(acc);
#pragma unroll
                for (int c = 0; c < NCH; ++c) {
                    uint4 af[4];
#pragma unroll
                    for (int i = 0; i < 4; ++i) {
                        const int row = nb * 64 + i * 16 + (l & 15);
                        af[i] = *reinterpret_cast<const uint4*>(smem + row * RL + ((c * 64 + ((l >> 4) << 4)) ^ swz(row)));
                    }
#pragma unroll
                    for (int i = 0; i < 4; ++i) {
#pragma unroll
                        for (int mt = 0; mt < MTS; ++mt) mma_chunk<T>(acc[i][mt], af[i], xf[mt][c]);
                    }
                }
                if (nb == nnb - 1 && strip + stride < strips) issue_x(strip + stride);
                if constexpr (EXT == 0 && sizeof(T) == 2) {
                    if (a.staged == 0) {
                        char* mine = smem + (size_t)bnp * RL + (size_t)bnp * 4 + wave * (16 * EPI_LD);
                        const int rsub = l >> 3, cb = (l & 7) * 16;
                        const int ncol = n_blk + nb * 64 + (l & 7) * 8;
#pragma unroll
                        for (int mt = 0; mt < MTS; ++mt) {
                            char* rowp = mine + (l & 15) * EPI_LD + ((l >> 4) << 3);
#pragma unroll
                            for (int i = 0; i < 4; ++i) {
                                const f32x4 v = acc[i][mt] + *reinterpret_cast<const f32x4*>(sbias + nb * 64 + i * 16 + ((l >> 4) << 2));
                                *reinterpret_cast<uint2*>(rowp + i * 32) = make_uint2(pack_bf2(v[0], v[1]), pack_bf2(v[2], v[3]));
                            }
                            __builtin_amdgcn_fence(__ATOMIC_RELEASE, "wavefront");
                            asm volatile("s_waitcnt lgkmcnt(0)" ::: "memory");
                            __builtin_amdgcn_fence(__ATOMIC_ACQUIRE, "wavefront");
#pragma unroll
                            for (int it = 0; it < 2; ++it) {
                                const int r = it * 8 + rsub, m = strip * (16 * MTS) + mt * 16 + r;
                                const uint4 v = *reinterpret_cast<const uint4*>(mine + r * EPI_LD + cb);
#ifdef FW_STREAM_DBG
                                if ((a.dbg & 1) && v.x != 0x12345678u) continue;
#endif
                                if (m < a.M && ncol < a.N) *reinterpret_cast<uint4*>(a.C + ((long)m * a.ldc + ncol) * 2) = v;
                            }
                            __builtin_amdgcn_fence(__ATOMIC_RELEASE, "wavefront");
                            asm volatile("s_waitcnt lgkmcnt(0)" ::: "memory");
                            __builtin_amdgcn_fence(__ATOMIC_ACQUIRE, "wavefront");
                        }
                        continue;
                    }
                }
#pragma unroll
                for (int mt = 0; mt < MTS; ++mt) {
                    const int m = m_lane + mt * 16;
                    const int mc = m < a.M ? m : a.M - 1;
                    uint4 ext[4];
                    if constexpr (EXT != 0) {
#pragma unroll
                        for (int i = 0; i < 4; ++i) {
                            const int n0 = n_blk + nb * 64 + i * 16 + ((l >> 4) << 2);
                            epi_fetch<T>(a, ext[i], mc, n0 < a.N ? n0 : 0, 0);
                        }
                    }
#pragma unroll
                    for (int i = 0; i < 4; ++i) {
                        const int n0 = n_blk + nb * 64 + i * 16 + ((l >> 4) << 2);
#ifdef FW_STREAM_DBG
                        if ((a.dbg & 1) && acc[i][mt][0] != 12345.678f) continue;
#endif
                        if (m < a.M && n0 < a.N) epi_apply<T>(a, *reinterpret_cast<const f32x4*>(sbias + (n0 - n_blk)), ext[i], acc[i][mt], m, n0, rs[mt], 0);
                    }
                }
            }
        }
    }
}

template <typename T, int NCH, bool WT, int EXT>
int launch_stream(const GemmArgs& a, hipStream_t st) {
    constexpr int RL = NCH * 64;
    const bool stg = EXT == 0 && sizeof(T) == 2 && a.staged == 0;
    const size_t stage_b = stg ? (size_t)8 * 16 * EPI_LD : 0;
    const int maxb = (int)(((stg ? 60 * 1024 : 64 * 1024)) / RL) & ~63;
    const int ny = fw_cdiv(a.N, maxb);
    const int bnp = fw_cdiv(fw_cdiv(a.N, ny), 64) * 64;
    const size_t lds = (size_t)bnp * RL + (size_t)bnp * 4 + stage_b;
    FW_SET_LDS_ONCE((gemm_stream_kernel<T, NCH, WT, EXT>), 80 * 1024);
    int hot = 0;
    constexpr long LD_MAX = 1L << 24;
    const bool tail16 = a.N % 64 == 0 || a.N % 64 >= 16;
    if (sizeof(T) == 2 && STREAM_HOT(NCH, EXT) && a.alpha == 1.0f && !a.C2 && !a.accumulate && !a.c_zstride && a.ldx < LD_MAX && a.ldc < LD_MAX && a.ldaux < LD_MAX && a.ldr < LD_MAX) {
        if (EXT == 0) hot = stg;
        if (EXT == 1) hot = tail16 && a.act == 2 && !a.out_f32 && !a.rowscale && !a.residual;
        if (EXT == 2) hot = tail16 && a.act == 0 && a.out_f32 && a.residual != nullptr;
    }
#ifdef FW_STREAM_DBG
    if (a.dbg) hot = 0;
#endif
    const int strips = fw_cdiv(a.M, 16 * STREAM_MTS(NCH, EXT));
    int gx = fw_cdiv(strips, 8);
    static const int resident = [] {
        int per_cu = 0, dev = 0;
        hipDeviceProp_t prop;
        if (hipOccupancyMaxActiveBlocksPerMultiprocessor(&per_cu, gemm_stream_kernel<T, NCH, WT, EXT>, 512, 80 * 1024) != hipSuccess || per_cu < 1) per_cu = 1;
        if (hipGetDevice(&dev) != hipSuccess || hipGetDeviceProperties(&prop, dev) != hipSuccess) return 256 * per_cu;
        return prop.multiProcessorCount * per_cu;
    }();
    const int cap = resident / ny > 0 ? resident / ny : 1;
    if (gx > cap) gx = cap;
    FW_KNAME("gemm_stream_kernel<%s,%d,%s,%d>", tname<T>(), NCH, FW_B(WT), EXT);
    hipLaunchKernelGGL((gemm_stream_kernel<T, NCH, WT, EXT>), dim3(gx, ny), dim3(512), lds, st, a, bnp, hot);
    FW_LAUNCH_RET();
}

template <typename T, int NCH>
int dispatch_stream_n(const GemmArgs& a, int wt, hipStream_t st) {
    const int ext = a.act == 2 ? 1 : (a.residual != nullptr ? 2 : 0);
    if (wt) return ext == 1 ? launch_stream<T, NCH, true, 1>(a, st) : ext == 2 ? launch_stream<T, NCH, true, 2>(a, st) : launch_stream<T, NCH, true, 0>(a, st);
    return ext == 1 ? launch_stream<T, NCH, false, 1>(a, st) : ext == 2 ? launch_stream<T, NCH, false, 2>(a, st) : launch_stream<T, NCH, false, 0>(a, st);
}
template <typename T>
int dispatch_stream(const GemmArgs& a, int wt, hipStream_t st) {
    const int nch = fw_cdiv(a.K * TT<T>::SZ, 128) * 2;
    if (nch <= 2) return dispatch_stream_n<T, 2>(a, wt, st);
    if (nch <= 4) return dispatch_stream_n<T, 4>(a, wt, st);
    return dispatch_stream_n<T, 8>(a, wt, st);
}

template <typename T, int BN, bool XT, bool WT, bool GX, bool GW>
int launch(const GemmArgs& a, hipStream_t st) {
    const size_t lds = 2 * (size_t)(BM + BN) * LDS_ROW;
    FW_SET_LDS_ONCE((gemm_kernel<T, BN, XT, WT, GX, GW>), lds);
    dim3 grid(fw_cdiv(a.M, BM), fw_cdiv(a.N, BN), a.splitk);
    FW_KNAME("gemm_kernel<%s,%d,%s,%s,%s,%s>", tname<T>(), BN, FW_B(XT), FW_B(WT), FW_B(GX), FW_B(GW));
    hipLaunchKernelGGL((gemm_kernel<T, BN, XT, WT, GX, GW>), grid, dim3(256), lds, st, a);
    FW_LAUNCH_RET();
}

template <typename T, int BN>
int dispatch_trans(const GemmArgs& a, int xt, int wt, hipStream_t st) {
    const int kt = 128 / TT<T>::SZ;
    const bool whole = a.K % kt == 0;
    const bool gx = !xt && whole && a.x_op == 0, gw = !wt && whole && a.w_op == 0;
    if (!xt && !wt) {
        const int kt64 = 64 / TT<T>::SZ;
        if constexpr (BN == 128) {
            if (a.x_op == 0 && a.w_op == 0 && a.K % kt64 == 0 && !whole) return launch_ring64<T, BN, 3>(a, st);
        }
        if (gx && gw) {
            constexpr int RING3_MIN_STEPS = 28;
            if constexpr (BN == 64) {
                if (a.kper >= RING3_MIN_STEPS * kt) return launch_ring<T, BN, 3>(a, st);
            }
            return launch_ring<T, BN, 2>(a, st);
        }
        if (gx) return launch<T, BN, false, false, true, false>(a, st);
        if (gw) return launch<T, BN, false, false, false, true>(a, st);
        return launch<T, BN, false, false, false, false>(a, st);
    }
    if (!xt && wt) return gx ? launch<T, BN, false, true, true, false>(a, st) : launch<T, BN, false, true, false, false>(a, st);
    if (xt && !wt) return gw ? launch<T, BN, true, false, false, true>(a, st) : launch<T, BN, true, false, false, false>(a, st);
    return launch<T, BN, true, true, false, false>(a, st);
}

}

extern "C" int fw_gemm_last_kernel(char* buf, int n) {
    if (!buf || n <= 0) return -1;
    snprintf(buf, (size_t)n, "%s", g_last_kernel);
    return (int)strlen(g_last_kernel);
}

extern "C" int fw_wgrad_group_prob_bytes(void) { return (int)sizeof(GemmArgs); }
namespace {
__global__ void wgrad_group_fill_kernel(const long long* __restrict__ tab, GemmArgs* __restrict__ probs, int nprob) {
    const int i = blockIdx.x * blockDim.x + threadIdx.x;
    if (i >= nprob) return;
    const long long* t = tab + (size_t)i * 16;
    GemmArgs a;
    a.X = reinterpret_cast<const char*>(t[0]); a.W = reinterpret_cast<const char*>(t[1]); a.C = reinterpret_cast<char*>(t[2]);
    a.ldx = t[3]; a.ldw = t[4]; a.ldc = t[5]; a.M = (int)t[6]; a.N = (int)t[7]; a.K = (int)t[8]; a.kper = (int)t[9]; a.splitk = (int)t[10];
    a.x_op = a.w_op = 0; a.bias = nullptr; a.act = 0; a.slope = 0.f; a.aux = nullptr; a.ldaux = 0; a.rowscale = nullptr; a.rows_per_scale = 1;
    a.residual = nullptr; a.ldr = 0; a.out_f32 = 1; a.accumulate = (int)t[14]; a.C2 = nullptr; a.ldc2 = 0;
    a.xsum = reinterpret_cast<float*>(t[11]); a.c_zstride = t[12]; a.xsum_zstride = t[13]; a.alpha = 1.0f; a.staged = -1; a.dbg = 0;
    probs[i] = a;
}
}
extern "C" int fw_wgrad_group(const void* tab, void* probs, int nprob, const void* items, int nitems, int tile, void* stream) {
    FW_CHECK_ARG(tab && probs && items && nprob > 0 && nitems > 0 && (tile == 128 || tile == 256));
    hipStream_t st = (hipStream_t)stream;
    hipLaunchKernelGGL(wgrad_group_fill_kernel, dim3((nprob + 63) / 64), dim3(64), 0, st, (const long long*)tab, (GemmArgs*)probs, nprob);
    if (tile == 128) {
        const size_t lds = (size_t)3 * (32 * 256 + 32 * 256);
        FW_SET_LDS_ONCE(gemm_wgrad_group_kernel, lds);
        hipLaunchKernelGGL(gemm_wgrad_group_kernel, dim3(nitems), dim3(256), lds, st, (const GemmArgs*)probs, (const int4*)items);
    } else {
        const size_t lds = (size_t)3 * 4 * 32 * 256;
        FW_SET_LDS_ONCE(gemm_wgrad_group_big_kernel, lds);
        hipLaunchKernelGGL(gemm_wgrad_group_big_kernel, dim3(nitems), dim3(512), lds, st, (const GemmArgs*)probs, (const int4*)items);
    }
    FW_LAUNCH_RET();
}

extern "C" int fw_gemm(int dtype, const void* X, long ldx, int x_trans, int x_op, const void* W, long ldw,
                       int w_trans, int w_op, void* C, long ldc, int out_f32, int accumulate, int M, int N,
                       int K, float alpha, const float* bias, int act, float slope, const void* aux,
                       long ldaux, const float* rowscale, int rows_per_scale, const float* residual,
                       long ldr, int splitk, void* C2, long ldc2, float* xsum, long c_zstride, long xsum_zstride,
                       void* stream) {
    const int sz = dtype == FW_DT_BF16 ? 2 : 4;
    const int e16 = 16 / sz;
    FW_CHECK_ARG(dtype == FW_DT_F32 || dtype == FW_DT_BF16);
    FW_CHECK_ARG(M > 0 && N > 0 && K > 0 && X && W && C);
    FW_CHECK_ARG(N % 4 == 0);
    FW_CHECK_ARG(ldx % e16 == 0 && ldw % e16 == 0 && ldc % 4 == 0);
    const int csz = (out_f32 || dtype == FW_DT_F32) ? 4 : 2;
    FW_CHECK_ARG(((uintptr_t)X & 15) == 0 && ((uintptr_t)W & 15) == 0 && ((uintptr_t)C & (4 * csz - 1)) == 0);
    if (!x_trans) FW_CHECK_ARG((K * sz) % 4 == 0 && ldx >= K); else FW_CHECK_ARG(ldx >= M);
    if (!w_trans) FW_CHECK_ARG((K * sz) % 4 == 0 && ldw >= K); else FW_CHECK_ARG(ldw >= N);
    FW_CHECK_ARG(!accumulate || out_f32 || dtype == FW_DT_F32);
    FW_CHECK_ARG(splitk >= 1 && (splitk == 1 || accumulate || c_zstride > 0));
    FW_CHECK_ARG(c_zstride == 0 || (out_f32 && c_zstride % 4 == 0));
    FW_CHECK_ARG(act >= 0 && act <= 3 && (act != 2 || aux));
    FW_CHECK_ARG(!rowscale || rows_per_scale > 0);
    if (bias) FW_CHECK_ARG(((uintptr_t)bias & 15) == 0);
    if (residual) FW_CHECK_ARG(((uintptr_t)residual & 15) == 0 && ldr % 4 == 0);
    const int kt = 128 / sz;
    GemmArgs a;
    a.X = (const char*)X; a.W = (const char*)W; a.C = (char*)C;
    a.ldx = ldx; a.ldw = ldw; a.ldc = ldc; a.M = M; a.N = N; a.K = K;
    a.x_op = x_op; a.w_op = w_op; a.bias = bias; a.act = act; a.slope = slope;
    a.aux = (const char*)aux; a.ldaux = ldaux; a.rowscale = rowscale; a.rows_per_scale = rows_per_scale;
    a.residual = residual; a.ldr = ldr;
    a.out_f32 = (out_f32 || dtype == FW_DT_F32) ? 1 : 0;
    a.accumulate = accumulate;
    a.splitk = splitk;
    a.C2 = (char*)C2; a.ldc2 = ldc2; a.xsum = xsum; a.c_zstride = c_zstride; a.xsum_zstride = xsum_zstride;
    FW_CHECK_ARG(!xsum || x_trans);
    FW_CHECK_ARG(!C2 || (((uintptr_t)C2 & (4 * sz - 1)) == 0 && ldc2 % 4 == 0));
    a.kper = fw_cdiv(fw_cdiv(K, kt), splitk) * kt;
    a.alpha = alpha;
    a.staged = staged_mode(a);
    static const int dbg = getenv("FW_GEMM_BIG_DBG") ? atoi(getenv("FW_GEMM_BIG_DBG")) : 0;
    a.dbg = dbg;
    hipStream_t st = (hipStream_t)stream;
    const bool bf16 = dtype == FW_DT_BF16, no_ops = x_op == 0 && w_op == 0;
    const bool pl = plain_epilogue(a);
    const long tiles128 = (long)fw_cdiv(M, 128) * fw_cdiv(N, 128) * splitk;
    constexpr int STREAM_MIN_M = 32768;
    if (!x_trans && splitk == 1 && !accumulate && no_ops && !xsum && K * sz <= 512 && M >= STREAM_MIN_M)
        return bf16 ? dispatch_stream<bf16raw>(a, w_trans, st) : dispatch_stream<float>(a, w_trans, st);
    constexpr long BIG_MIN_TILES = 160;
    if (bf16 && !x_trans && no_ops && !xsum && splitk == 1 && !accumulate && K % 64 == 0 && K >= 256 &&
        ldx % 8 == 0 && ldw % 8 == 0 && (long)fw_cdiv(M, 256) * fw_cdiv(N, 256) >= BIG_MIN_TILES)
        return w_trans ? launch_big<true>(a, st) : launch_big<false>(a, st);
    const bool tr = bf16 && w_trans && no_ops && (N > 64 || (x_trans && N >= 8)) && K % 64 == 0 && a.kper % 64 == 0 && ldw % 8 == 0;
    if (tr && x_trans && ldx % 8 == 0) return launch_tr_ring<true, 32, 3>(a, st);
    constexpr long TR_MIN_TILES = 200;
    if (tr && !x_trans && !xsum && tiles128 >= TR_MIN_TILES) {
        if (pl && tiles128 > 256) return launch_tr_ring<false, 32, 3>(a, st);
        return pl ? launch_tr_ring<false, 64, 3>(a, st) : launch_tr_ring<false, 64, 2>(a, st);
    }
    constexpr long TR_K32_MIN_TILES = 200;
    if (bf16 && w_trans && !x_trans && no_ops && N > 64 && K % 64 != 0 && K % 32 == 0 && ldw % 8 == 0 && !xsum
        && splitk == 1 && tiles128 >= TR_K32_MIN_TILES)
        return launch_tr_ring<false, 32, 3>(a, st);
    constexpr long BN128_MIN_TILES = 384;
    const bool small_n = N <= 64 || tiles128 < BN128_MIN_TILES;
    if (bf16) return small_n ? dispatch_trans<bf16raw, 64>(a, x_trans, w_trans, st) : dispatch_trans<bf16raw, 128>(a, x_trans, w_trans, st);
    return small_n ? dispatch_trans<float, 64>(a, x_trans, w_trans, st) : dispatch_trans<float, 128>(a, x_trans, w_trans, st);
}
```

### frequency-wised_all-in-one_image_restoration_model_amd/fwair/ops.py

```python
import bisect

import torch

from . import lfs as _lfs
from .lib import call, dt, lib


def _ld(t):
    assert t.dim() == 2 and t.stride(1) == 1, 'expect a row-major 2-D view'
    return t.stride(0)


def empty(rows, cols, dtype, device):
    return torch.empty((rows, cols), dtype=dtype, device=device)


def gemm(x, w, M, N, K, *, x_trans=False, w_trans=False, x_op=0, w_op=0, out=None, out_dtype=None, bias=None,
         act=0, slope=0.0, aux=None, rowscale=None, rows_per_scale=1, residual=None, accumulate=False, splitk=1,
         alpha=1.0, out_gelu=None, xsum=None, c_zstride=0, xsum_zstride=0):
    assert x.dtype == w.dtype
    if out is None:
        out = torch.empty((M, N), dtype=out_dtype or x.dtype, device=x.device)
    if accumulate:
        _note_write(out)
    if xsum is not None and not xsum_zstride:
        _note_write(xsum)
    out_f32 = int(out.dtype == torch.float32)
    call('fw_gemm', dt(x.dtype), x, _ld(x), int(x_trans), x_op, w, _ld(w), int(w_trans), w_op, out, _ld(out), out_f32,
         int(accumulate), M, N, K, float(alpha), bias, act, float(slope), aux, _ld(aux) if aux is not None else 0,
         rowscale, rows_per_scale, residual, _ld(residual) if residual is not None else 0, splitk,
         out_gelu, _ld(out_gelu) if out_gelu is not None else 0, xsum, c_zstride, xsum_zstride)
    return out


import os as _os
_SPLITK_BLOCKS = int(_os.environ.get('FW_SPLITK_BLOCKS', '512'))
_DGRAD_SPLIT_ROWS = int(_os.environ.get('FW_DGRAD_SPLIT_ROWS', '512'))


def pick_splitk(M, N, K, dtype):
    tiles = ((M + 127) // 128) * ((N + 63) // 64 if N <= 64 else (N + 127) // 128)
    sk = max(1, min(_SPLITK_BLOCKS // max(tiles, 1), K // 512))
    while sk > 1 and sk * M * N * 4 > (256 << 20):
        sk //= 2
    return int(sk)


_zeroed = []
_zeroed_bufs = {}


def _span(t):
    lo = t.data_ptr()
    if t.numel() == 0:
        return lo, lo
    return lo, lo + t.element_size() * (1 + sum((n - 1) * st for n, st in zip(t.shape, t.stride())))


def _clusters(spans):
    order = sorted(range(len(spans)), key=lambda i: spans[i][0])
    union, shared, first = [], [False] * len(spans), 0
    for i in order:
        lo, hi = spans[i]
        if lo >= hi:
            continue
        if union and lo < union[-1][1]:
            union[-1][1] = max(union[-1][1], hi)
            shared[first] = shared[i] = True
        else:
            union.append([lo, hi])
            first = i
    return union, shared


def mark_zeroed(t):
    assert t.is_contiguous()
    lo, hi = _span(t)
    _unmark([(lo, hi)])
    _zeroed.append((lo, hi))
    _zeroed.sort()
    _zeroed_bufs[lo] = t
    for p in [p for p, b in _zeroed_bufs.items() if not any(z[0] < _span(b)[1] and _span(b)[0] < z[1] for z in _zeroed)]:
        del _zeroed_bufs[p]


def clear_marks():
    _zeroed.clear()
    _zeroed_bufs.clear()


def _unmark(spans):
    if not _zeroed or not spans:
        return
    cut, out, j = _clusters(spans)[0], [], 0
    for lo, hi in _zeroed:
        while j < len(cut) and cut[j][1] <= lo:
            j += 1
        cur, k = lo, j
        while k < len(cut) and cut[k][0] < hi:
            if cut[k][0] > cur:
                out.append((cur, cut[k][0]))
            cur = max(cur, cut[k][1])
            k += 1
        if cur < hi:
            out.append((cur, hi))
    _zeroed[:] = out


def _note_write(t):
    if _zeroed and t is not None:
        lo, hi = _span(t)
        i = bisect.bisect_left(_zeroed, (hi,))
        if i and _zeroed[i - 1][1] > lo:
            _unmark([(lo, hi)])


def _is_zero(span):
    i = bisect.bisect_right(_zeroed, (span[0], float('inf')))
    return i > 0 and _zeroed[i - 1][0] <= span[0] and span[1] <= _zeroed[i - 1][1]


_pending = []
_flush_registered = [None]
_keepalive = []


_HOST_WORDS = 65536
_host_ring, _host_next, _host_reserved = [], [0], []


def reserve_capture_tables(count=None):
    if count is None:
        count = 6
    while len(_host_reserved) < count:
        _host_reserved.append(torch.empty((_HOST_WORDS,), dtype=torch.int64, pin_memory=True))


def _host_table(words):
    assert words <= _HOST_WORDS, 'too many pending slabs for one table'
    if torch.cuda.is_current_stream_capturing():
        if not _host_reserved:
            raise RuntimeError('fwair.ops: call reserve_capture_tables() before capturing a backward pass')
        buf = _host_reserved.pop()
        _keepalive.append(buf)
        return buf[:words]
    if len(_host_ring) < 4:
        _host_ring.append([torch.empty((_HOST_WORDS,), dtype=torch.int64, pin_memory=True), None])
    slot = _host_ring[_host_next[0] % len(_host_ring)]
    _host_next[0] += 1
    if slot[1] is not None:
        slot[1].synchronize()
    slot[1] = torch.cuda.Event()
    return slot[0][:words]


def _in_backward():
    return torch._C._current_graph_task_id() != -1


def slab_reduce(slab, nz, n, zstride, dst, dst2=None, off2=0, n2=0, defer=False):
    _note_write(dst)
    _note_write(dst2)
    if not defer or not _in_backward():
        call('fw_slab_reduce', slab, nz, n, zstride, dst, 1, dst2, off2, n2 if dst2 is not None else 0)
        return
    _register_flush()
    _pending.append((slab, nz, n, zstride, dst, dst2, off2, n2 if dst2 is not None else 0))


def flush_slabs():
    _flush_registered[0] = None
    try:
        _flush_wgrads()
        _fold_slabs()
    except BaseException:
        _pending.clear(); _pending_w.clear(); clear_marks()
        raise


def _fold_slabs():
    if not _pending:
        return
    items = list(_pending)
    _pending.clear()
    num = len(items)
    dev = items[0][0].device
    host = _host_table(num * 12 + num + 1)
    tab, prefix = host[:num * 12].view(num, 12), host[num * 12:]
    rows, offs, total = [], [0], 0
    spans, owner = [], []
    for i, it in enumerate(items):
        spans.append(_span(it[4])); owner.append(i)
        if it[5] is not None:
            spans.append(_span(it[5])); owner.append(i)
    shared_item = [False] * num
    for i, sh in zip(owner, _clusters(spans)[1]):
        shared_item[i] |= sh
    for (slab, nz, n, zstride, dst, dst2, off2, n2), shared in zip(items, shared_item):
        end = off2 + n2 if dst2 is not None else n
        nchunks = ((end + 3) // 4 + 63) // 64
        zper = min(nz, 64)
        splits = (nz + zper - 1) // zper
        upw = max(1, 32 // zper)
        blocks = (nchunks * splits + 4 * upw - 1) // (4 * upw)
        unaligned = dst.data_ptr() % 16 or (dst2 is not None and dst2.data_ptr() % 16)
        rows.append((slab.data_ptr(), dst.data_ptr(), dst2.data_ptr() if dst2 is not None else 0, n, zstride, off2, n2, nz, zper,
                     nchunks, upw, int(splits > 1 or shared or bool(unaligned))))
        total += blocks
        offs.append(total)
    tab.copy_(torch.tensor(rows, dtype=torch.int64))
    prefix.copy_(torch.tensor(offs, dtype=torch.int64))
    table = torch.empty(host.shape, dtype=torch.int64, device=dev)
    table.copy_(host, non_blocking=True)
    call('fw_slab_reduce_multi', table, table[num * 12:], num, total)
    if not torch.cuda.is_current_stream_capturing():
        for slot in _host_ring:
            if slot[0].data_ptr() == host.data_ptr():
                slot[1].record()


_GROUP = int(_os.environ.get('FW_WGRAD_GROUP', '1'))
_GROUP_CHUNK = int(_os.environ.get('FW_WGRAD_CHUNK', '4096'))
_GROUP_BIG_MIN = int(_os.environ.get('FW_WGRAD_BIG_MIN', '224'))
_GROUP_PLAIN = int(_os.environ.get('FW_WGRAD_PLAIN', '1'))
_GROUP_UNIT_BX = int(_os.environ.get('FW_WGRAD_UNIT_BX', '1'))
_pending_w = []
_dw_mode = {}


def _register_flush():
    task = torch._C._current_graph_task_id()
    if _flush_registered[0] != task:
        if _flush_registered[0] is not None:
            _pending.clear(); _pending_w.clear()
        _flush_registered[0] = task
        torch.autograd.Variable._execution_engine.queue_callback(flush_slabs)


def _groupable(g, x, n, k, m, dw, db):
    return (_GROUP and g.dtype == torch.bfloat16 and x.dtype == torch.bfloat16 and m % 32 == 0 and g.stride(1) == 1 and x.stride(1) == 1
            and g.stride(0) % 8 == 0 and x.stride(0) % 8 == 0 and g.data_ptr() % 16 == 0 and x.data_ptr() % 16 == 0 and n >= 8 and k % 4 == 0
            and dw.dtype == torch.float32 and dw.stride(1) == 1 and dw.stride(0) % 4 == 0 and dw.data_ptr() % 16 == 0)


def _flush_wgrads():
    if not _pending_w:
        return
    work = list(_pending_w)
    _pending_w.clear()
    spans = [_span(w_[5]) for w_ in work]
    shared = _clusters(spans)[1]
    unsliced = [i for i, w_ in enumerate(work) if w_[4] <= _GROUP_CHUNK]
    racing = _clusters([spans[i] for i in unsliced])[1]
    _dw_mode.clear()
    for i, r in zip(unsliced, racing):
        _dw_mode[spans[i]] = 2 if r else 1 if shared[i] or not _GROUP_PLAIN or not _is_zero(spans[i]) else 0
    _unmark(spans + [_span(w_[6]) for w_ in work if w_[6] is not None])
    big = [w for w in work if min(w[2], w[3]) >= _GROUP_BIG_MIN]
    small = [w for w in work if min(w[2], w[3]) < _GROUP_BIG_MIN]
    if big:
        _launch_group(big, 256)
    if small:
        _launch_group(small, 128)


def _group_fire(table, probs, nprob, total, tile):
    call('fw_wgrad_group', table, probs, nprob, table[nprob * 16:], total, tile)


def _launch_group(work, tile=128):
    dev = work[0][0].device
    rows, units = [], []
    for pi, (g, x, n, k, m, dw, db) in enumerate(work):
        tm, tn = (n + tile - 1) // tile, (k + tile - 1) // tile
        sk = max(1, -(-m // _GROUP_CHUNK))
        kper = -(-(-(-m // sk)) // 32) * 32
        sk = -(-m // kper)
        if sk == 1:
            mode = _dw_mode.get(_span(dw), 2)
            rows.append((g.data_ptr(), x.data_ptr(), dw.data_ptr(), g.stride(0), x.stride(0), dw.stride(0), n, k, m, kper, 1,
                         db.data_ptr() if db is not None else 0, 1 if mode == 0 else 0, 0, mode, 0))
        else:
            nk = (n * k + 3) // 4 * 4
            S = nk + (n + 3) // 4 * 4
            slab = torch.empty((sk, S), dtype=torch.float32, device=dev)
            rows.append((g.data_ptr(), x.data_ptr(), slab.data_ptr(), g.stride(0), x.stride(0), k, n, k, m, kper, sk,
                         slab.data_ptr() + 4 * nk if db is not None else 0, S, S if db is not None else 0, 0, 0))
            assert dw.is_contiguous() or dw.stride(0) == k
            _pending.append((slab, sk, n * k, S, dw, db, nk, n if db is not None else 0))
        for z in range(sk):
            for bx in range(0, tm, _GROUP_UNIT_BX):
                units.append((min(kper, m - z * kper), pi, bx, min(_GROUP_UNIT_BX, tm - bx), tn, z))
    units.sort(key=lambda u: -u[0])
    lists, load = [[] for _ in range(8)], [0] * 8
    for ln, pi, bx, u, tn, z in units:
        x = load.index(min(load))
        load[x] += ln * tn * u
        lists[x].extend((pi, bx + i, by, z) for by in range(tn) for i in range(u))
    depth = max(len(li) for li in lists)
    total = depth * 8
    items = [lists[p & 7][p >> 3] if (p >> 3) < len(lists[p & 7]) else (-1, 0, 0, 0) for p in range(total)]
    nprob = len(rows)
    words = nprob * 16 + total * 2
    if words > _HOST_WORDS and len(work) > 1:
        del _pending[len(_pending) - sum(1 for r_ in rows if r_[10] > 1):]
        _launch_group(work[:len(work) // 2], tile); _launch_group(work[len(work) // 2:], tile)
        return
    host = _host_table(words)
    host[:nprob * 16].view(nprob, 16).copy_(torch.tensor(rows, dtype=torch.int64))
    it32 = torch.tensor(items, dtype=torch.int32)
    host[nprob * 16:].view(torch.int32).view(total, 4).copy_(it32)
    table = torch.empty(host.shape, dtype=torch.int64, device=dev)
    table.copy_(host, non_blocking=True)
    probs = torch.empty(nprob * lib().fw_wgrad_group_prob_bytes(), dtype=torch.uint8, device=dev)
    _group_fire(table, probs, nprob, total, tile)
    if not torch.cuda.is_current_stream_capturing():
        for slot in _host_ring:
            if slot[0].data_ptr() == host.data_ptr():
                slot[1].record()


def wgrad(g, x, n, k, m, dw, db=None, defer=False):
    if defer and _in_backward() and _groupable(g, x, n, k, m, dw, db):
        _register_flush()
        _pending_w.append((g, x, n, k, m, dw, db))
        return
    _note_write(dw)
    _note_write(db)
    sk = pick_splitk(n, k, m, g.dtype)
    if sk == 1:
        gemm(g, x, n, k, m, x_trans=True, w_trans=True, out=dw, accumulate=True, xsum=db)
        return
    nk = (n * k + 3) // 4 * 4
    S = nk + (n + 3) // 4 * 4
    slab = torch.empty((sk, S), dtype=torch.float32, device=g.device)
    cview = slab[0, :n * k].view(n, k)
    xs = slab[0, nk:] if db is not None else None
    gemm(g, x, n, k, m, x_trans=True, w_trans=True, out=cview, splitk=sk, xsum=xs, c_zstride=S, xsum_zstride=S if db is not None else 0)
    slab_reduce(slab, sk, n * k, S, dw, db, nk, n, defer=defer)


def dgrad(g, w, M, K, N, out, act=0, aux=None):
    tiles = ((M + 127) // 128) * ((K + 127) // 128)
    sk = min(512 // max(tiles, 1), N // _DGRAD_SPLIT_ROWS) if (act == 0 and tiles < 200) else 1
    if sk <= 1:
        gemm(g, w, M, K, N, w_trans=True, out=out, act=act, aux=aux)
        return
    S = (M * K + 3) // 4 * 4
    slab = torch.empty((sk, S), dtype=torch.float32, device=g.device)
    gemm(g, w, M, K, N, w_trans=True, out=slab[0, :M * K].view(M, K), splitk=sk, c_zstride=S)
    direct = out.dtype == torch.float32 and out.is_contiguous()
    tmp = out if direct else torch.empty((M, K), dtype=torch.float32, device=g.device)
    call('fw_slab_reduce', slab, sk, M * K, S, tmp, 0, None, 0, 0)
    if not direct:
        call('fw_cast_rows', dt(out.dtype), tmp, K, out, _ld(out), M, K, None, 1)


def layernorm_fwd(x, gamma, beta, out_dtype, eps=1e-5):
    rows, C = x.shape
    y = torch.empty((rows, C), dtype=out_dtype, device=x.device)
    mean = torch.empty(rows, dtype=torch.float32, device=x.device)
    rstd = torch.empty(rows, dtype=torch.float32, device=x.device)
    call('fw_layernorm_fwd', dt(out_dtype), x, _ld(x), gamma, beta, y, _ld(y), mean, rstd, rows, C, eps)
    return y, mean, rstd


def layernorm_bwd(dy, x, gamma, mean, rstd, dgamma, dbeta, dres=None, defer=False, twin=None, twscale=None, tw_rows_per_scale=1):
    rows, C = x.shape
    dx = torch.empty((rows, C), dtype=torch.float32, device=x.device)
    nblk = lib().fw_layernorm_bwd_blocks(rows, C)
    partial = torch.empty((nblk, 2 * C), dtype=torch.float32, device=x.device)
    call('fw_layernorm_bwd2', dt(dy.dtype), dy, _ld(dy), x, _ld(x), gamma, mean, rstd, dres,
         _ld(dres) if dres is not None else 0, dx, _ld(dx), None, None, partial, rows, C,
         twin, _ld(twin) if twin is not None else 0, twscale, tw_rows_per_scale)
    slab_reduce(partial, nblk, C, 2 * C, dgamma, dbeta, C, C, defer=defer)
    return dx


def attn_fwd(qkv, C, B, H, W, heads, L, mode, shift, bias, coef=None, lfs=0):
    rows = qkv.shape[0]
    D = C // heads
    nkt = 1 if mode == 0 else L - 1
    out = torch.empty((rows, C), dtype=qkv.dtype, device=qkv.device)
    nitems = B * (H // 8) * (W // 8) * L * heads
    lse = torch.empty((nitems, 64), dtype=torch.float32, device=qkv.device)
    tab = _lfs.device_table(qkv.dtype, qkv.device) if lfs == 2 else None
    call('fw_attn_fwd', dt(qkv.dtype), D, nkt, lfs, qkv, qkv[:, C:], qkv[:, 2 * C:], _ld(qkv), out, _ld(out), lse, bias,
         coef, tab, B, H, W, heads, L, mode, shift, float(D) ** -0.5)
    return out, lse


def attn_bwd(qkv, out, dout, lse, C, B, H, W, heads, L, mode, shift, bias, dbias_dense, coef=None, dcoef=None, lfs=0):
    rows = qkv.shape[0]
    D = C // heads
    nkt = 1 if mode == 0 else L - 1
    dqkv = torch.empty_like(qkv)
    d2 = torch.empty_like(qkv) if nkt == 2 else None
    _note_write(dbias_dense)
    _note_write(dcoef)
    tab = _lfs.device_table(qkv.dtype, qkv.device) if lfs == 2 else None
    call('fw_attn_bwd', dt(qkv.dtype), D, nkt, lfs, qkv, qkv[:, C:], qkv[:, 2 * C:], _ld(qkv), out, _ld(out), dout, _ld(dout),
         lse, bias, coef, tab, dqkv, dqkv[:, C:], dqkv[:, 2 * C:], d2[:, C:] if d2 is not None else None,
         d2[:, 2 * C:] if d2 is not None else None, _ld(dqkv),
         dbias_dense, dcoef, B, H, W, heads, L, mode, shift, float(D) ** -0.5, 0)
    if nkt == 2:
        call('fw_add_rows', dt(qkv.dtype), d2[:, C:], _ld(d2), dqkv[:, C:], _ld(dqkv), rows, 2 * C)
    return dqkv


def rel_index(device):
    ch = torch.arange(8)
    coords = torch.stack(torch.meshgrid([ch, ch], indexing='ij')).flatten(1)
    rel = (coords[:, :, None] - coords[:, None, :]).permute(1, 2, 0).contiguous()
    rel[:, :, 0] += 7
    rel[:, :, 1] += 7
    rel[:, :, 0] *= 15
    return rel.sum(-1).to(device)


def dwconv_fwd(src, w, bias, B, H, W, in_gelu=False):
    h2, g2 = torch.empty_like(src), torch.empty_like(src)
    call('fw_dwconv_fwd', dt(src.dtype), src, _ld(src), int(in_gelu), w, bias, h2, g2, _ld(h2), B, H, W, src.shape[1])
    return h2, g2


def dwconv_bwd(dh2, g1, h1, w, dw, dbias, B, H, W):
    dh1 = torch.empty_like(h1)
    _note_write(dw)
    _note_write(dbias)
    call('fw_dwconv_bwd', dt(h1.dtype), dh2, _ld(dh2), g1, h1, _ld(h1), w, dh1, _ld(dh1), dw, dbias, B, H, W, h1.shape[1])
    return dh1


def im2col4(x, B, H, W, dtype):
    C = x.shape[1]
    col = torch.empty((B * (H // 2) * (W // 2), 16 * C), dtype=dtype, device=x.device)
    call('fw_im2col4', dt(dtype), x, _ld(x), col, B, H, W, C)
    return col


def col2im4(dcol, B, H, W, C, dres=None):
    dx = torch.empty((B * H * W, C), dtype=torch.float32, device=dcol.device)
    call('fw_col2im4', dt(dcol.dtype), dcol, dx, _ld(dx), dres, _ld(dres) if dres is not None else 0, B, H, W, C)
    return dx


def pixel_shuffle(g, bias, out, B, H, W, Cout):
    call('fw_pixel_shuffle', dt(g.dtype), g, bias, out, _ld(out), B, H, W, Cout)
    return out


def pixel_unshuffle(dout, B, H, W, Cout, dtype):
    dg = torch.empty((B * H * W, 4 * Cout), dtype=dtype, device=dout.device)
    call('fw_pixel_unshuffle', dt(dtype), dout, _ld(dout), dg, B, H, W, Cout)
    return dg


def colsum(x, out):
    _note_write(out)
    call('fw_colsum', 1 if x.dtype == torch.bfloat16 else 0, x, _ld(x), out, x.shape[0], x.shape[1])


def cast_rows(src, dtype, rowscale=None, rows_per_scale=1):
    dst = torch.empty(src.shape, dtype=dtype, device=src.device)
    call('fw_cast_rows', dt(dtype), src, _ld(src), dst, _ld(dst), src.shape[0], src.shape[1], rowscale, rows_per_scale)
    return dst


def copy_rows(src, dst, accumulate=False):
    if accumulate:
        _note_write(dst)
    call('fw_copy_rows', src, _ld(src), dst, _ld(dst), src.shape[0], src.shape[1], int(accumulate))


def permute3(src, dst, dims, out_strides, accumulate=False):
    ind = 1 if src.dtype == torch.bfloat16 else 0
    outd = 1 if dst.dtype == torch.bfloat16 else 0
    if accumulate:
        _note_write(dst)
    call('fw_permute3', ind, outd, src, dst, dims[0], dims[1], dims[2], out_strides[0], out_strides[1], out_strides[2],
         int(accumulate))
```

### include/fwair.h

```cpp
#ifndef FWAIR_H
#define FWAIR_H
#ifdef __cplusplus
extern "C" {
#endif

int fw_gemm(int dtype, const void* X, long ldx, int x_trans, int x_op, const void* W, long ldw, int w_trans, int w_op,
            void* C, long ldc, int out_f32, int accumulate, int M, int N, int K, float alpha, const float* bias, int act,
            float slope, const void* aux, long ldaux, const float* rowscale, int rows_per_scale, const float* residual,
            long ldr, int splitk, void* C2, long ldc2, float* xsum, long c_zstride, long xsum_zstride, void* stream);
int fw_gemm_last_kernel(char* buf, int n);

int fw_wgrad_group_prob_bytes(void);
int fw_wgrad_group(const void* tab, void* probs, int nprob, const void* items, int nitems, int tile, void* stream);

int fw_slab_reduce(const float* slab, int nz, long n, long zstride, float* dst, int accumulate, float* dst2, long off2, long n2,
                   void* stream);
int fw_slab_reduce_multi(const void* tab, const void* prefix, int num, long total_blocks, void* stream);

int fw_layernorm_fwd(int dtype, const float* x, long ldx, const float* gamma, const float* beta, void* y, long ldy,
                     float* mean, float* rstd, int rows, int C, float eps, void* stream);
int fw_layernorm_bwd_blocks(int rows, int C);
int fw_layernorm_bwd(int dtype, const void* dy, long lddy, const float* x, long ldx, const float* gamma, const float* mean,
                     const float* rstd, const float* dres, long lddres, float* dx, long lddx, float* dgamma, float* dbeta,
                     float* partial, int rows, int C, void* stream);
int fw_layernorm_bwd2(int dtype, const void* dy, long lddy, const float* x, long ldx, const float* gamma, const float* mean,
                      const float* rstd, const float* dres, long lddres, float* dx, long lddx, float* dgamma, float* dbeta,
                      float* partial, int rows, int C, void* twin, long ldtw, const float* twscale, int tw_rows_per_scale,
                      void* stream);

int fw_attn_lfs_table_elems(void);
int fw_attn_fwd(int dtype, int D, int nkt, int lfs, const void* q, const void* k, const void* v, long ld, void* out, long ldo,
                float* lse, const float* bias, const float* coef, const void* lfs_tab, int B, int H, int W, int heads, int L,
                int mode, int shift, float scale, void* stream);
int fw_attn_bwd(int dtype, int D, int nkt, int lfs, const void* q, const void* k, const void* v, long ld, const void* out,
                long ldo, const void* dout, long lddo, const float* lse, const float* bias, const float* coef,
                const void* lfs_tab, void* dq, void* dk, void* dv, void* dk2, void* dv2, long ldd, float* dbias,
                float* dcoef, int B, int H, int W, int heads, int L, int mode, int shift, float scale, int dq_pad, void* stream);

int fw_dwconv_fwd(int dtype, const void* in, long ld1, int in_gelu, const float* w, const float* bias, void* h2, void* g2, long ld2, int B,
                  int H, int W, int C, void* stream);
int fw_dwconv_bwd(int dtype, const void* dh2, long ldg, const void* g1, const void* h1, long ld1, const float* w, void* dh1,
                  long ldo, float* dw, float* dbias, int B, int H, int W, int C, void* stream);

int fw_im2col4(int dtype, const float* x, long ldx, void* col, int B, int H, int W, int C, void* stream);
int fw_col2im4(int dtype, const void* dcol, float* dx, long lddx, const float* dres, long ldr, int B, int H, int W, int C,
               void* stream);
int fw_pixel_shuffle(int dtype, const void* g, const float* bias, float* out, long ldo, int B, int H, int W, int Cout,
                     void* stream);
int fw_pixel_unshuffle(int dtype, const float* dout, long ldo, void* dg, int B, int H, int W, int Cout, void* stream);
int fw_colsum(int x_dtype, const void* x, long ldx, float* out, long rows, int cols, void* stream);

int fw_inproj_fwd(const float* img, const float* w, const float* bias, float* out, long ldo, int B, int H, int W, int C,
                  float slope, void* stream);
int fw_inproj_bwd(const float* img, const float* out, long ldo, const float* dy, long ldy, float* dw, float* db, int B, int H,
                  int W, int C, float slope, void* stream);
int fw_outproj_fwd(const float* fea, long ldf, const float* w, const float* bias, const float* img, float* out, int B, int H,
                   int W, int C, void* stream);
int fw_outproj_bwd(const float* dout, const float* fea, long ldf, const float* w, float* dfea, long lddf, float* dw, float* db,
                   int B, int H, int W, int C, void* stream);

int fw_cast_rows(int dtype, const float* src, long lds_, void* dst, long ldd, long rows, int cols, const float* rowscale,
                 int rows_per_scale, void* stream);
int fw_copy_rows(const float* src, long lds_, float* dst, long ldd, long rows, int cols, int accumulate, void* stream);
int fw_add_rows(int dtype, const void* src, long lds_, void* dst, long ldd, long rows, int cols, void* stream);
int fw_cast_flat(int dtype, const float* src, void* dst, long n, void* stream);
int fw_permute3(int in_dtype, int out_dtype, const void* in, void* out, int d0, int d1, int d2, long s0, long s1, long s2,
                int accumulate, void* stream);
int fw_permute3_multi(const void* tab, const void* prefix, int num, long total_blocks, void* stream);
int fw_fill(float* p, long n, float v, void* stream);
int fw_lrelu_fwd(int dtype, const float* x, void* y, long n, float slope, void* stream);
int fw_lrelu_bwd(int dtype, const void* dy, const float* x, float* dx, long n, float slope, void* stream);

int fw_l1_loss(const float* a, const float* b, float* da, long n, float gscale, float* loss, void* stream);
int fw_ce0_loss(const float* logits, float* dlogits, int R, int N, float gscale, float* loss, void* stream);

int fw_adam_tick(float* hyper, float b1, float b2, void* stream);
int fw_adam(int shadow_dtype, float* p, const float* g, float* m, float* v, void* shadow, long n, const float* hyper, float b1,
            float b2, float eps, void* stream);
int fw_ema(int shadow_dtype, float* pk, const float* pq, void* shadow, long n, float momentum, void* stream);

int fw_dft2_fwd(const float* img, float* fr, float* fi, int nimg, int N, void* stream);
int fw_dft2_bands(const float* fr, const float* fi, const float* mask_unshifted, float* out, int nimg, int N, int nbands,
                  int mode, void* stream);
int fw_dft2_decompose(const float* img, const float* mask, const float* panels, float* out, int nimg, int N, int nbands, int dc_bits,
                      void* stream);
int fw_band_residual(const float* img, float* out, int nimg, int N, int nbands, void* stream);
int fw_dc_split(const float* img, float* out, int nimg, int NN, void* stream);
int fw_dft2t_fwd(const float* img, const float* panels, float* work, float* fr, float* fi, int nimg, int N, void* stream);
int fw_dft2t_bands(const float* fr, const float* fi, const float* mask_unshifted, const float* panels, float* work, float* out,
                   int nimg, int N, int nbands, int mode, void* stream);
int fw_dft2t_decompose(const float* img, const float* mask, const float* panels, float* work, float* out, int nimg, int N,
                       int nbands, int dc_bits, void* stream);

int fw_bn_lrelu_gap_fwd(int dtype, const void* fea, const float* gamma, const float* beta, float* rmean, float* rvar,
                        long long* nbt, float* part, float* saved, float* gap, int B, int ED, int P, int training, float eps,
                        float momentum, float slope, void* stream);
int fw_bn_lrelu_gap_bwd(int dtype, const void* fea, const float* gamma, const float* beta, const float* saved, const float* dgap,
                        float* part2, void* dfea, float* dgamma, float* dbeta, int B, int ED, int P, float slope, void* stream);

int fw_moco_logits(const float* q, const float* k, const float* queue, float* logits, float* khat, int L, int B, int ED, int K,
                   float invT, void* stream);
int fw_moco_logits_bwd(const float* q, const float* khat, const float* queue, const float* dlogits, float* dq, int L, int B,
                       int ED, int K, float invT, void* stream);
int fw_moco_enqueue(float* queue, const float* khat, long long* ptr, int L, int B, int ED, int K, void* stream);

int fw_lfs_xbar(const float* inter, float* xbar, float* stats, int nb1, int B, int NT, int C, float eps, void* stream);
int fw_lfs_xbar_bwd(const float* inter, const float* stats, const float* dxbar, float* dinter, int nb1, int B, int NT, int C,
                    void* stream);
int fw_lfs_lambda(const float* xbar, const unsigned long long* ptab, const int* heads, const long long* coef_off, float* coef,
                  float* save, int nblk, int B, int C, int nb1, void* stream);
int fw_lfs_lambda_bwd(const float* xbar, const unsigned long long* ptab, const unsigned long long* gtab, const int* heads,
                      const long long* coef_off, const float* dcoef, const float* save, float* dxbar, int nblk, int B, int C,
                      int nb1, void* stream);

int fw_conv3x3(int dtype, const void* x, long ldx, const void* x2, long ldx2, int cin, int cin1, const void* w, const float* bias,
               void* out, long ldo, int out_f32, const void* res, long ldr, int cout, int B, int H, int W, int stride, int taps,
               int act, float slope, void* stream);
int fw_im2col3(int dtype, const void* x, long ldx, void* col, int B, int H, int W, int C, int stride, void* stream);
int fw_col2im3(int dtype, const void* dcol, void* dx, long lddx, int B, int H, int W, int C, int stride, void* stream);
int fw_dcn_im2col(int dtype, const void* x, long ldx, const float* om, void* col, int B, int H, int W, int C, void* stream);
int fw_dcn_bwd(int dtype, const void* dcol, const void* x, long ldx, const float* om, float* dx, long lddx, float* dom, int B, int H,
               int W, int C, void* stream);
int fw_bn_cl_fwd(int dtype, const void* x, long ldx, const float* gamma, const float* beta, float* rmean, float* rvar, long long* nbt,
                 float* sums, float* mr, const void* res, long ldr, void* y, long ldy, long rows, int C, int training, float eps,
                 float momentum, float slope, void* stream);
int fw_bn_cl_bwd(int dtype, const void* dy, long ldd, const void* y, long ldy, const void* x, long ldx, const float* mr,
                 const float* gamma, float* sums, void* dx, long lddx, void* dres, long lddr, long rows, int C, int training,
                 float slope, void* stream);
int fw_lrelu_t(int dtype, const void* x, long ldx, void* y, long ldy, long rows, int C, float slope, void* stream);
int fw_lrelu_t_bwd(int dtype, const void* dy, long ldd, const void* y, long ldy, void* dx, long lddx, long rows, int C, float slope,
                   void* stream);
int fw_dgm_fwd(int dtype, const void* x, const void* dcn, const void* gamma, const void* beta, void* out, long n, float slope,
               void* stream);
int fw_dgm_bwd(int dtype, const void* dout, const void* out, const void* x, const void* gamma, void* dx, void* dz, void* dgamma,
               long n, float slope, void* stream);
int fw_gap_cl(int dtype, const void* x, long ldx, float* out, int B, int P, int C, void* stream);
int fw_gap_cl_bwd(int dtype, const float* dgap, void* dx, long lddx, int B, int P, int C, void* stream);
int fw_nchw_to_tokens(int dtype, const float* img, void* tok, long ld, int B, int Ci, int HW, int Cp, void* stream);
int fw_tokens_to_nchw(int dtype, const void* tok, long ld, float* img, int B, int Ci, int HW, void* stream);

int fw_add_bcast(const float* x, const float* p, float* out, long n, long period, void* stream);
int fw_bn_planes_fwd(int dtype, const void* fea, const float* gamma, const float* beta, float* rmean, float* rvar, long long* nbt, float* mr,
                     float* inter, float* gap, int B, int ED, int P, int training, float eps, float momentum, float slope, void* stream);
int fw_bn_planes_bwd(int dtype, const void* fea, const float* inter, const float* gamma, const float* mr, const float* dinter,
                     const float* dgap, void* dfea, float* dgamma, float* dbeta, int B, int ED, int P, int training, float slope,
                     void* stream);
int fw_small_linear_fwd(const float* x, const float* w, const float* b, float* y, int M, int N, int K, float slope, void* stream);
int fw_small_linear_bwd(const float* dy, const float* y, const float* x, const float* w, float* dx, float* dw, float* db, int M, int N,
                        int K, float slope, void* stream);

int fw_gattn_fwd(int dtype, const void* q, const void* k, const void* v, long ld, void* out, long ldo, float* lse, int B, int heads, int N,
                 float scale, const void* seed, int site, float drop_p, const float* lamb, int nb, int lamb_batch, const void* bandidx,
                 const float* panels, void* stream);
int fw_gattn_bwd(int dtype, const void* q, const void* k, const void* v, long ld, const void* o, long ldo, const void* dout, long lddo,
                 const float* lse, float* dvec, void* dq, void* dk, void* dv, long ldd, int B, int heads, int N, float scale,
                 const void* seed, int site, float drop_p, const float* lamb, float* dlamb, int nb, int lamb_batch, const void* bandidx,
                 const float* panels, void* stream);
int fw_gattn_bands_fwd(int dtype, const void* q, const void* k, const void* v, long ld, void* out, long ldo, float* lse, int B, int heads,
                       float scale, const void* seed, int site, float drop_p, const float* lamb, int nb, int lamb_batch, const void* bandidx,
                       const float* panels, float* amap, float* work, void* stream);
int fw_gattn_bands_bwd(int dtype, const void* q, const void* k, const void* v, long ld, const void* dout, long lddo, const float* lse,
                       float* dvec, void* dq, void* dk, void* dv, long ldd, int B, int heads, float scale, const void* seed, int site,
                       float drop_p, const float* lamb, float* dlamb, int nb, int lamb_batch, const void* bandidx, const float* panels,
                       const float* amap, float* pmap, float* gmap, float* work, void* stream);
int fw_gattn_bandsn_fwd(int dtype, const void* q, const void* k, const void* v, long ld, void* out, long ldo, float* lse, int B, int heads,
                        int N, float scale, const void* seed, int site, float drop_p, const float* lamb, int nb, int lamb_batch,
                        const void* bandidx, const float* panels, float* amap, float* work, void* stream);
int fw_gattn_bandsn_bwd(int dtype, const void* q, const void* k, const void* v, long ld, const void* dout, long lddo, const float* lse,
                        float* dvec, void* dq, void* dk, void* dv, long ldd, int B, int heads, int N, float scale, const void* seed,
                        int site, float drop_p, const float* lamb, float* dlamb, int nb, int lamb_batch, const void* bandidx,
                        const float* panels, const float* amap, float* pmap, float* gmap, float* work, void* stream);
int fw_dropout(int mode, int dtype, const void* x, const void* aux, const float* res, void* y, long n, long period, const void* seed, int site,
               float p, void* stream);
int fw_rng_tick(void* seed, void* stream);

int fw_train_batch(const void* tab, const int* rnd, const float* sigma, const void* seed, int site, float* d1, float* d2, float* c1,
                   float* c2, int B, int S, void* stream);
int fw_tile_gather(const float* img, const int* ys, const int* xs, float* tiles, int C, int H, int W, int ny, int nx, int T, void* stream);
int fw_tile_blend(const float* tiles, const int* ys, const int* xs, float* out, int C, int H, int W, int ny, int nx, int T, void* stream);
int fw_ssim7(const float* a, const float* b, float* out, int n, int C, int H, int W, void* stream);
int fw_eval_gather(const void* itab, const int* ttab, const float* sigma, const void* seed, int site, float* tiles, int N, int T,
                   void* stream);
int fw_eval_blend(const void* itab, const void* gtab, const int* ttab, const float* rest, float* packed, void* u8out, float* sse,
                  int i0, int nimg, int ntiles, int T, void* stream);
int fw_eval_ssim7(const void* itab, const void* gtab, const float* packed, float* out, int i0, int nimg, void* stream);

int fw_leff_fwd(const void* xn, long ldx, const void* w1p, const float* b1, const float* wd, const float* bd, const void* w2p,
                const float* b2, const float* res, long ldr, const float* rowscale, int rows_per_scale, float* y, long ldy, void* h1,
                void* g1, void* h2, void* g2, long ldh, int B, int H, int W, int C, void* stream);

#ifdef __cplusplus
}
#endif
#endif
```

Before: 345.1 images/sec.

## Add fused in-kernel split-K with last-arriver reduction and auto split selection

Adds split-K variants of the bf16 GEMM kernels. Each z-slice writes its fp32 partial accumulators to a persistent workspace and bumps a per-tile atomic counter. The last block to arrive sums all slices and runs the normal epilogue, so the separate slab-reduce and cast kernels and their launches go away. A heuristic picks the split factor automatically for low-tile, large-K GEMMs, and dgrad now routes through this path, including the GELU-aux case. The cost is extra global traffic for the partials, a counter protocol that depends on correct memory ordering, and a workspace shared per stream.

```diff
diff --git a/frequency-wised_all-in-one_image_restoration_model_amd/csrc/fw_gemm.hip b/frequency-wised_all-in-one_image_restoration_model_amd/csrc/fw_gemm.hip
--- a/frequency-wised_all-in-one_image_restoration_model_amd/csrc/fw_gemm.hip
+++ b/frequency-wised_all-in-one_image_restoration_model_amd/csrc/fw_gemm.hip
@@ -28,6 +28,8 @@
     float alpha;
     int staged;
     int dbg;
+    float* sk_ws; unsigned* sk_cnt; int sk_n;
+    long sk_ws_bytes; int sk_ncnt;
 };
 
 constexpr int LDS_ROW = 128;
@@ -37,6 +39,68 @@
 FW_DEV unsigned xcd_contiguous(unsigned lin, unsigned total) {
     const unsigned xcd = lin & 7, q = total >> 3, r = total & 7;
     return (xcd < r ? xcd * (q + 1) : r * (q + 1) + (xcd - r) * q) + (lin >> 3);
+}
+
+FW_DEV void sk_remap(int& bx, int& by, int& bz) {
+    const unsigned total = gridDim.x * gridDim.y * gridDim.z;
+    const unsigned lin = blockIdx.x + gridDim.x * (blockIdx.y + gridDim.y * blockIdx.z);
+    const unsigned w = xcd_contiguous(lin, total);
+    const unsigned t = w / gridDim.z;
+    bz = (int)(w % gridDim.z);
+    bx = (int)(t % gridDim.x);
+    by = (int)(t / gridDim.x);
+}
+template <int WM>
+FW_DEV bool splitk_combine(const GemmArgs& a, f32x4 (&acc)[4][WM], int bx, int by, int bz, char* smem) {
+    constexpr int NF = 4 * WM;
+    constexpr size_t SLICE = (size_t)NF * 256;
+    const int nz = a.sk_n, tid = threadIdx.x;
+    const unsigned tile = (unsigned)by * gridDim.x + (unsigned)bx;
+    f32x4* base = reinterpret_cast<f32x4*>(a.sk_ws) + (size_t)tile * nz * SLICE + tid;
+    f32x4* mine = base + (size_t)bz * SLICE;
+#pragma unroll
+    for (int mt = 0; mt < WM; ++mt)
+#pragma unroll
+        for (int nt = 0; nt < 4; ++nt)
+            asm volatile("global_store_dwordx4 %0, %1, off sc1\n\ts_nop 1" ::"v"(mine + (mt * 4 + nt) * 256), "v"(acc[nt][mt]) : "memory");
+    asm volatile("s_waitcnt vmcnt(0)" ::: "memory");
+    __syncthreads();
+    volatile unsigned* flag = reinterpret_cast<volatile unsigned*>(smem);
+    if (tid == 0) {
+        const unsigned ticket = __hip_atomic_fetch_add(a.sk_cnt + tile, 1u, __ATOMIC_RELAXED, __HIP_MEMORY_SCOPE_AGENT);
+        const unsigned last = ticket == (unsigned)(nz - 1) ? 1u : 0u;
+        if (last) {
+            __hip_atomic_store(a.sk_cnt + tile, 0u, __ATOMIC_RELAXED, __HIP_MEMORY_SCOPE_AGENT);
+            __builtin_amdgcn_fence(__ATOMIC_ACQUIRE, "agent");
+            asm volatile("s_waitcnt vmcnt(0)" ::: "memory");
+        }
+        *flag = last;
+    }
+    __syncthreads();
+    if (*flag == 0u) return false;
+#pragma unroll
+    for (int mt = 0; mt < WM; ++mt) {
+        f32x4 s[4][4];
+        zero_acc(s);
+        for (int z0 = 0; z0 < nz; z0 += 4) {
+            f32x4 t[4][4];
+#pragma unroll
+            for (int w = 0; w < 4; ++w) {
+                const f32x4* p = base + (size_t)min(z0 + w, nz - 1) * SLICE + (mt * 4) * 256;
+#pragma unroll
+                for (int nt = 0; nt < 4; ++nt) t[w][nt] = p[nt * 256];
+            }
+#pragma unroll
+            for (int w = 0; w < 4; ++w)
+                if (z0 + w < nz) {
+#pragma unroll
+                    for (int nt = 0; nt < 4; ++nt) s[w][nt] += t[w][nt];
+                }
+        }
+#pragma unroll
+        for (int nt = 0; nt < 4; ++nt) acc[nt][mt] = s[0][nt] + ((s[1][nt] + s[2][nt]) + s[3][nt]);
+    }
+    return true;
 }
 
 template <typename T> FW_DEV uint4 apply_gelu16(const uint4& v) {
@@ -245,18 +309,18 @@
     return *reinterpret_cast<const uint4*>(tile + row * LDS_ROW + ((chunk * 64 + ((l >> 4) << 4)) ^ swz(row)));
 }
 
-template <typename T, int BN, bool XT, bool WT, bool GX, bool GW>
-__global__ __launch_bounds__(256) void gemm_kernel(GemmArgs a) {
+template <typename T, int BN, bool XT, bool WT, bool GX, bool GW, bool SK>
+FW_DEV void gemm_tile(const GemmArgs a, char* smem) {
     constexpr int KT = 128 / TT<T>::SZ;
     constexpr int WM = (BN == 128) ? 4 : 2;
     constexpr int XBYTES = BM * LDS_ROW, WBYTES = BN * LDS_ROW;
-    extern __shared__ __attribute__((aligned(16))) char smem[];
     auto xs = [&](int i) -> char* { return smem + i * (XBYTES + WBYTES); };
     auto ws = [&](int i) -> char* { return smem + i * (XBYTES + WBYTES) + XBYTES; };
 
     const int wave = threadIdx.x >> 6;
     int bx = blockIdx.x, by = blockIdx.y, bz = blockIdx.z;
-    {
+    if constexpr (SK) sk_remap(bx, by, bz);
+    else {
         const unsigned total = gridDim.x * gridDim.y * gridDim.z;
         if (gridDim.z > 1) {
             const unsigned lin = blockIdx.x + gridDim.x * (blockIdx.y + gridDim.y * blockIdx.z);
@@ -345,6 +409,10 @@
             }
         }
     }
+    if constexpr (SK) {
+        if (!splitk_combine<WM>(a, acc, bx, by, bz, smem)) return;
+        bz = 0;
+    }
     const int l = lane_id();
     f32x4 bias4[4];
 #pragma unroll
@@ -369,6 +437,16 @@
             if (m < a.M && n0 < a.N) epi_apply<T>(a, bias4[nt], ext[nt], acc[nt][mt], m, n0, rs, bz);
         }
     }
+}
+template <typename T, int BN, bool XT, bool WT, bool GX, bool GW>
+__global__ __launch_bounds__(256) void gemm_kernel(GemmArgs a) {
+    extern __shared__ __attribute__((aligned(16))) char smem[];
+    gemm_tile<T, BN, XT, WT, GX, GW, false>(a, smem);
+}
+template <typename T, int BN, bool WT, bool GX, bool GW>
+__global__ __launch_bounds__(256, 2) void gemm_kernel_sk(GemmArgs a) {
+    extern __shared__ __attribute__((aligned(16))) char smem[];
+    gemm_tile<T, BN, false, WT, GX, GW, true>(a, smem);
 }
 
 FW_DEV int swz256(int r) { return ((r & 3) << 2) | ((r >> 2) & 3); }
@@ -542,6 +620,10 @@
         }
     }
 }
+static inline bool sk_fits(const GemmArgs& a, int bn) {
+    const long tiles = (long)fw_cdiv(a.M, 128) * fw_cdiv(a.N, bn);
+    return a.sk_ws && a.sk_cnt && tiles <= (long)a.sk_ncnt && tiles * a.sk_n * (128L * bn * 4) <= a.sk_ws_bytes;
+}
 static inline bool plain_epilogue(const GemmArgs& a) {
     return a.act == 0 && !a.rowscale && !a.residual && !a.C2 && a.alpha == 1.0f && !(a.accumulate && a.c_zstride == 0);
 }
@@ -702,7 +784,7 @@
     return -1;
 }
 
-template <bool XT, int KT, int NS, bool PLAIN>
+template <bool XT, int KT, int NS, bool PLAIN, bool SK = false>
 FW_DEV void tr_ring_tile(const GemmArgs& a, int bx, int by, int bz, char* smem) {
     using T = bf16raw;
     static_assert(NS == 2 || NS == 3, "ring depth");
@@ -779,6 +861,10 @@
                 else atomicAdd(a.xsum + m, xsacc[n][0]);
             }
         }
+    }
+    if constexpr (SK) {
+        if (!splitk_combine<WM>(a, acc, bx, by, bz, smem)) return;
+        bz = 0;
     }
     if (a.staged >= 0 && (size_t)NS * STAGE >= (size_t)4 * 16 * WM * EPI_LD) {
         __syncthreads();
@@ -812,6 +898,13 @@
     }
     tr_ring_tile<XT, KT, NS, PLAIN>(a, bx, by, bz, smem);
 }
+template <int KT, int NS, bool PLAIN>
+__global__ __launch_bounds__(256, 2) void gemm_tr_ring_kernel_sk(GemmArgs a) {
+    extern __shared__ __attribute__((aligned(16))) char smem[];
+    int bx, by, bz;
+    sk_remap(bx, by, bz);
+    tr_ring_tile<false, KT, NS, PLAIN, true>(a, bx, by, bz, smem);
+}
 
 __global__ __launch_bounds__(256, 3) void gemm_wgrad_group_kernel(const GemmArgs* __restrict__ probs, const int4* __restrict__ items) {
     extern __shared__ __attribute__((aligned(16))) char smem[];
@@ -921,6 +1014,15 @@
 template <bool XT, int KT, int NS, bool PLAIN>
 int launch_tr_ring_p(const GemmArgs& a, hipStream_t st) {
     const size_t lds = (size_t)NS * ((XT ? KT * 256 : 128 * ((KT == 32) ? ROW64 : LDS_ROW)) + KT * 256);
+    if constexpr (!XT) {
+        if (a.sk_n > 1) {
+            FW_CHECK_ARG(sk_fits(a, 128));
+            FW_SET_LDS_ONCE((gemm_tr_ring_kernel_sk<KT, NS, PLAIN>), lds);
+            FW_KNAME("gemm_tr_ring_kernel<%s,%d,%d,%s>", FW_B(XT), KT, NS, FW_B(PLAIN));
+            hipLaunchKernelGGL((gemm_tr_ring_kernel_sk<KT, NS, PLAIN>), dim3(fw_cdiv(a.M, 128), fw_cdiv(a.N, 128), a.sk_n), dim3(256), lds, st, a);
+            FW_LAUNCH_RET();
+        }
+    }
     FW_SET_LDS_ONCE((gemm_tr_ring_kernel<XT, KT, NS, PLAIN>), lds);
     FW_KNAME("gemm_tr_ring_kernel<%s,%d,%d,%s>", FW_B(XT), KT, NS, FW_B(PLAIN));
     hipLaunchKernelGGL((gemm_tr_ring_kernel<XT, KT, NS, PLAIN>), dim3(fw_cdiv(a.M, 128), fw_cdiv(a.N, 128), a.splitk), dim3(256), lds, st, a);
@@ -931,18 +1033,18 @@
     return plain_epilogue(a) ? launch_tr_ring_p<XT, KT, NS, true>(a, st) : launch_tr_ring_p<XT, KT, NS, false>(a, st);
 }
 
-template <typename T, int BN, int NS, bool PLAIN>
-__global__ __launch_bounds__(256) void gemm_ring_kernel(GemmArgs a) {
+template <typename T, int BN, int NS, bool PLAIN, bool SK>
+FW_DEV void gemm_ring_tile(const GemmArgs a, char* smem) {
     constexpr int KT = 128 / TT<T>::SZ;
     constexpr int WM = (BN == 128) ? 4 : 2;
     constexpr int XBYTES = BM * LDS_ROW, WBYTES = BN * LDS_ROW, STAGE = XBYTES + WBYTES;
     constexpr int LPS = BM / 32 + BN / 32;
-    extern __shared__ __attribute__((aligned(16))) char smem[];
     auto xs = [&](int i) -> char* { return smem + i * STAGE; };
     auto ws = [&](int i) -> char* { return smem + i * STAGE + XBYTES; };
     const int wave = threadIdx.x >> 6;
     int bx = blockIdx.x, by = blockIdx.y, bz = blockIdx.z;
-    {
+    if constexpr (SK) sk_remap(bx, by, bz);
+    else {
         const unsigned total = gridDim.x * gridDim.y * gridDim.z;
         if (gridDim.z > 1) {
             const unsigned lin = blockIdx.x + gridDim.x * (blockIdx.y + gridDim.y * blockIdx.z);
@@ -1002,6 +1104,10 @@
         }
         buf = buf + 1 == NS ? 0 : buf + 1;
     }
+    if constexpr (SK) {
+        if (!splitk_combine<WM>(a, acc, bx, by, bz, smem)) return;
+        bz = 0;
+    }
     if constexpr (sizeof(T) == 2) {
         if (a.staged >= 0 && (size_t)NS * STAGE >= (size_t)4 * 16 * WM * EPI_LD) {
             __syncthreads();
@@ -1013,8 +1119,28 @@
 }
 
 template <typename T, int BN, int NS, bool PLAIN>
+__global__ __launch_bounds__(256) void gemm_ring_kernel(GemmArgs a) {
+    extern __shared__ __attribute__((aligned(16))) char smem[];
+    gemm_ring_tile<T, BN, NS, PLAIN, false>(a, smem);
+}
+template <int BN, int NS, bool PLAIN>
+__global__ __launch_bounds__(256, 2) void gemm_ring_kernel_sk(GemmArgs a) {
+    extern __shared__ __attribute__((aligned(16))) char smem[];
+    gemm_ring_tile<bf16raw, BN, NS, PLAIN, true>(a, smem);
+}
+
+template <typename T, int BN, int NS, bool PLAIN>
 int launch_ring_p(const GemmArgs& a, hipStream_t st) {
     const size_t lds = (size_t)NS * (BM + BN) * LDS_ROW;
+    if constexpr (sizeof(T) == 2) {
+        if (a.sk_n > 1) {
+            FW_CHECK_ARG(sk_fits(a, BN));
+            FW_SET_LDS_ONCE((gemm_ring_kernel_sk<BN, NS, PLAIN>), lds);
+            FW_KNAME("gemm_ring_kernel<%s,%d,%d,%s>", tname<T>(), BN, NS, FW_B(PLAIN));
+            hipLaunchKernelGGL((gemm_ring_kernel_sk<BN, NS, PLAIN>), dim3(fw_cdiv(a.M, BM), fw_cdiv(a.N, BN), a.sk_n), dim3(256), lds, st, a);
+            FW_LAUNCH_RET();
+        }
+    }
     FW_SET_LDS_ONCE((gemm_ring_kernel<T, BN, NS, PLAIN>), lds);
     dim3 grid(fw_cdiv(a.M, BM), fw_cdiv(a.N, BN), a.splitk);
     FW_KNAME("gemm_ring_kernel<%s,%d,%d,%s>", tname<T>(), BN, NS, FW_B(PLAIN));
@@ -1026,19 +1152,19 @@
     return plain_epilogue(a) ? launch_ring_p<T, BN, NS, true>(a, st) : launch_ring_p<T, BN, NS, false>(a, st);
 }
 
-template <typename T, int BN, int NS, bool PLAIN>
-__global__ __launch_bounds__(256) void gemm_ring64_kernel(GemmArgs a) {
+template <typename T, int BN, int NS, bool PLAIN, bool SK>
+FW_DEV void gemm_ring64_tile(const GemmArgs a, char* smem) {
     constexpr int KT = ROW64 / TT<T>::SZ;
     constexpr int WM = (BN == 128) ? 4 : 2;
     constexpr int XBYTES = BM * ROW64, WBYTES = BN * ROW64, STAGE = XBYTES + WBYTES;
     constexpr int LPS = BM / 64 + BN / 64;
     static_assert(NS >= 3, "ring depth");
-    extern __shared__ __attribute__((aligned(16))) char smem[];
     auto xs = [&](int i) -> char* { return smem + i * STAGE; };
     auto ws = [&](int i) -> char* { return smem + i * STAGE + XBYTES; };
     const int wave = threadIdx.x >> 6;
     int bx = blockIdx.x, by = blockIdx.y, bz = blockIdx.z;
-    {
+    if constexpr (SK) sk_remap(bx, by, bz);
+    else {
         const unsigned total = gridDim.x * gridDim.y * gridDim.z;
         if (gridDim.z > 1) {
             const unsigned lin = blockIdx.x + gridDim.x * (blockIdx.y + gridDim.y * blockIdx.z);
@@ -1096,6 +1222,10 @@
             for (int n = 0; n < WM; ++n) mma_chunk<T>(acc[m][n], af[m], bfr[n]);
         buf = buf + 1 == NS ? 0 : buf + 1;
     }
+    if constexpr (SK) {
+        if (!splitk_combine<WM>(a, acc, bx, by, bz, smem)) return;
+        bz = 0;
+    }
     if constexpr (sizeof(T) == 2) {
         if (a.staged >= 0 && (size_t)NS * STAGE >= (size_t)4 * 16 * WM * EPI_LD) {
             __syncthreads();
@@ -1107,8 +1237,28 @@
 }
 
 template <typename T, int BN, int NS, bool PLAIN>
+__global__ __launch_bounds__(256) void gemm_ring64_kernel(GemmArgs a) {
+    extern __shared__ __attribute__((aligned(16))) char smem[];
+    gemm_ring64_tile<T, BN, NS, PLAIN, false>(a, smem);
+}
+template <int BN, int NS, bool PLAIN>
+__global__ __launch_bounds__(256, 2) void gemm_ring64_kernel_sk(GemmArgs a) {
+    extern __shared__ __attribute__((aligned(16))) char smem[];
+    gemm_ring64_tile<bf16raw, BN, NS, PLAIN, true>(a, smem);
+}
+
+template <typename T, int BN, int NS, bool PLAIN>
 int launch_ring64_p(const GemmArgs& a, hipStream_t st) {
     const size_t lds = (size_t)NS * (BM + BN) * ROW64;
+    if constexpr (sizeof(T) == 2) {
+        if (a.sk_n > 1) {
+            FW_CHECK_ARG(sk_fits(a, BN));
+            FW_SET_LDS_ONCE((gemm_ring64_kernel_sk<BN, NS, PLAIN>), lds);
+            FW_KNAME("gemm_ring64_kernel<%s,%d,%d,%s>", tname<T>(), BN, NS, FW_B(PLAIN));
+            hipLaunchKernelGGL((gemm_ring64_kernel_sk<BN, NS, PLAIN>), dim3(fw_cdiv(a.M, BM), fw_cdiv(a.N, BN), a.sk_n), dim3(256), lds, st, a);
+            FW_LAUNCH_RET();
+        }
+    }
     FW_SET_LDS_ONCE((gemm_ring64_kernel<T, BN, NS, PLAIN>), lds);
     dim3 grid(fw_cdiv(a.M, BM), fw_cdiv(a.N, BN), a.splitk);
     FW_KNAME("gemm_ring64_kernel<%s,%d,%d,%s>", tname<T>(), BN, NS, FW_B(PLAIN));
@@ -1862,6 +2012,15 @@
 template <typename T, int BN, bool XT, bool WT, bool GX, bool GW>
 int launch(const GemmArgs& a, hipStream_t st) {
     const size_t lds = 2 * (size_t)(BM + BN) * LDS_ROW;
+    if constexpr (sizeof(T) == 2 && !XT) {
+        if (a.sk_n > 1) {
+            FW_CHECK_ARG(sk_fits(a, BN));
+            FW_SET_LDS_ONCE((gemm_kernel_sk<T, BN, WT, GX, GW>), lds);
+            FW_KNAME("gemm_kernel<%s,%d,%s,%s,%s,%s>", tname<T>(), BN, FW_B(XT), FW_B(WT), FW_B(GX), FW_B(GW));
+            hipLaunchKernelGGL((gemm_kernel_sk<T, BN, WT, GX, GW>), dim3(fw_cdiv(a.M, BM), fw_cdiv(a.N, BN), a.sk_n), dim3(256), lds, st, a);
+            FW_LAUNCH_RET();
+        }
+    }
     FW_SET_LDS_ONCE((gemm_kernel<T, BN, XT, WT, GX, GW>), lds);
     dim3 grid(fw_cdiv(a.M, BM), fw_cdiv(a.N, BN), a.splitk);
     FW_KNAME("gemm_kernel<%s,%d,%s,%s,%s,%s>", tname<T>(), BN, FW_B(XT), FW_B(WT), FW_B(GX), FW_B(GW));
@@ -1915,6 +2074,7 @@
     a.x_op = a.w_op = 0; a.bias = nullptr; a.act = 0; a.slope = 0.f; a.aux = nullptr; a.ldaux = 0; a.rowscale = nullptr; a.rows_per_scale = 1;
     a.residual = nullptr; a.ldr = 0; a.out_f32 = 1; a.accumulate = (int)t[14]; a.C2 = nullptr; a.ldc2 = 0;
     a.xsum = reinterpret_cast<float*>(t[11]); a.c_zstride = t[12]; a.xsum_zstride = t[13]; a.alpha = 1.0f; a.staged = -1; a.dbg = 0;
+    a.sk_ws = nullptr; a.sk_cnt = nullptr; a.sk_n = 0; a.sk_ws_bytes = 0; a.sk_ncnt = 0;
     probs[i] = a;
 }
 }
@@ -1934,12 +2094,27 @@
     FW_LAUNCH_RET();
 }
 
-extern "C" int fw_gemm(int dtype, const void* X, long ldx, int x_trans, int x_op, const void* W, long ldw,
-                       int w_trans, int w_op, void* C, long ldc, int out_f32, int accumulate, int M, int N,
-                       int K, float alpha, const float* bias, int act, float slope, const void* aux,
-                       long ldaux, const float* rowscale, int rows_per_scale, const float* residual,
-                       long ldr, int splitk, void* C2, long ldc2, float* xsum, long c_zstride, long xsum_zstride,
-                       void* stream) {
+static int sk_auto(int M, int N, int K, long t128) {
+    constexpr long ROUND = 512, BN128_MIN = 384, IDLE_MAX = 128;
+    constexpr int MIN_K = 512, MAX_SK = 12;
+    int kmax = K / MIN_K;
+    if (kmax > MAX_SK) kmax = MAX_SK;
+    const long t64 = (long)fw_cdiv(M, 128) * fw_cdiv(N, 64);
+    if (kmax < 2 || t64 > IDLE_MAX || 2.0 * M * N * K < (double)(1 << 30)) return 1;
+    long sk = ROUND / t128 < kmax ? ROUND / t128 : kmax;
+    if (sk >= 2 && t128 * sk >= BN128_MIN) return (int)sk;
+    sk = ROUND / t64 < kmax ? ROUND / t64 : kmax;
+    return sk >= 2 ? (int)sk : 1;
+}
+static thread_local int g_auto_sk = 0;
+
+static int gemm_run(int dtype, const void* X, long ldx, int x_trans, int x_op, const void* W, long ldw,
+                    int w_trans, int w_op, void* C, long ldc, int out_f32, int accumulate, int M, int N,
+                    int K, float alpha, const float* bias, int act, float slope, const void* aux,
+                    long ldaux, const float* rowscale, int rows_per_scale, const float* residual,
+                    long ldr, int splitk, void* C2, long ldc2, float* xsum, long c_zstride, long xsum_zstride,
+                    void* sk_ws, long sk_ws_bytes, void* sk_cnt, int sk_ncnt, int fused, void* stream) {
+    g_auto_sk = 0;
     const int sz = dtype == FW_DT_BF16 ? 2 : 4;
     const int e16 = 16 / sz;
     FW_CHECK_ARG(dtype == FW_DT_F32 || dtype == FW_DT_BF16);
@@ -1951,7 +2126,12 @@
     if (!x_trans) FW_CHECK_ARG((K * sz) % 4 == 0 && ldx >= K); else FW_CHECK_ARG(ldx >= M);
     if (!w_trans) FW_CHECK_ARG((K * sz) % 4 == 0 && ldw >= K); else FW_CHECK_ARG(ldw >= N);
     FW_CHECK_ARG(!accumulate || out_f32 || dtype == FW_DT_F32);
-    FW_CHECK_ARG(splitk >= 1 && (splitk == 1 || accumulate || c_zstride > 0));
+    if (fused) {
+        FW_CHECK_ARG(dtype == FW_DT_BF16 && splitk >= 0 && !x_trans && !xsum && !accumulate && c_zstride == 0);
+        FW_CHECK_ARG(sk_ws_bytes >= 0 && sk_ncnt >= 0 && ((uintptr_t)sk_ws & 15) == 0 && ((uintptr_t)sk_cnt & 3) == 0);
+    } else {
+        FW_CHECK_ARG(splitk >= 1 && (splitk == 1 || accumulate || c_zstride > 0));
+    }
     FW_CHECK_ARG(c_zstride == 0 || (out_f32 && c_zstride % 4 == 0));
     FW_CHECK_ARG(act >= 0 && act <= 3 && (act != 2 || aux));
     FW_CHECK_ARG(!rowscale || rows_per_scale > 0);
@@ -1966,11 +2146,12 @@
     a.residual = residual; a.ldr = ldr;
     a.out_f32 = (out_f32 || dtype == FW_DT_F32) ? 1 : 0;
     a.accumulate = accumulate;
-    a.splitk = splitk;
+    a.splitk = fused ? 1 : splitk;
+    a.sk_ws = (float*)sk_ws; a.sk_cnt = (unsigned*)sk_cnt; a.sk_n = 0; a.sk_ws_bytes = sk_ws_bytes; a.sk_ncnt = sk_ncnt;
     a.C2 = (char*)C2; a.ldc2 = ldc2; a.xsum = xsum; a.c_zstride = c_zstride; a.xsum_zstride = xsum_zstride;
     FW_CHECK_ARG(!xsum || x_trans);
     FW_CHECK_ARG(!C2 || (((uintptr_t)C2 & (4 * sz - 1)) == 0 && ldc2 % 4 == 0));
-    a.kper = fw_cdiv(fw_cdiv(K, kt), splitk) * kt;
+    a.kper = fw_cdiv(fw_cdiv(K, kt), a.splitk) * kt;
     a.alpha = alpha;
     a.staged = staged_mode(a);
     static const int dbg = getenv("FW_GEMM_BIG_DBG") ? atoi(getenv("FW_GEMM_BIG_DBG")) : 0;
@@ -1978,14 +2159,25 @@
     hipStream_t st = (hipStream_t)stream;
     const bool bf16 = dtype == FW_DT_BF16, no_ops = x_op == 0 && w_op == 0;
     const bool pl = plain_epilogue(a);
-    const long tiles128 = (long)fw_cdiv(M, 128) * fw_cdiv(N, 128) * splitk;
     constexpr int STREAM_MIN_M = 32768;
-    if (!x_trans && splitk == 1 && !accumulate && no_ops && !xsum && K * sz <= 512 && M >= STREAM_MIN_M)
+    if (!x_trans && splitk <= 1 && !accumulate && no_ops && !xsum && K * sz <= 512 && M >= STREAM_MIN_M)
         return bf16 ? dispatch_stream<bf16raw>(a, w_trans, st) : dispatch_stream<float>(a, w_trans, st);
     constexpr long BIG_MIN_TILES = 160;
-    if (bf16 && !x_trans && no_ops && !xsum && splitk == 1 && !accumulate && K % 64 == 0 && K >= 256 &&
+    if (bf16 && !x_trans && no_ops && !xsum && splitk <= 1 && !accumulate && K % 64 == 0 && K >= 256 &&
         ldx % 8 == 0 && ldw % 8 == 0 && (long)fw_cdiv(M, 256) * fw_cdiv(N, 256) >= BIG_MIN_TILES)
         return w_trans ? launch_big<true>(a, st) : launch_big<false>(a, st);
+    int nz = splitk;
+    if (fused) {
+        const long t128 = (long)fw_cdiv(M, 128) * fw_cdiv(N, 128);
+        const int ksteps = fw_cdiv(K, kt);
+        if (splitk == 0) nz = sk_auto(M, N, K, t128);
+        if (nz > ksteps) nz = ksteps;
+        a.kper = fw_cdiv(ksteps, nz) * kt;
+        nz = fw_cdiv(K, a.kper);
+        a.sk_n = nz > 1 ? nz : 0;
+        if (splitk == 0 && nz > 1) g_auto_sk = nz;
+    }
+    const long tiles128 = (long)fw_cdiv(M, 128) * fw_cdiv(N, 128) * nz;
     const bool tr = bf16 && w_trans && no_ops && (N > 64 || (x_trans && N >= 8)) && K % 64 == 0 && a.kper % 64 == 0 && ldw % 8 == 0;
     if (tr && x_trans && ldx % 8 == 0) return launch_tr_ring<true, 32, 3>(a, st);
     constexpr long TR_MIN_TILES = 200;
@@ -1995,10 +2187,37 @@
     }
     constexpr long TR_K32_MIN_TILES = 200;
     if (bf16 && w_trans && !x_trans && no_ops && N > 64 && K % 64 != 0 && K % 32 == 0 && ldw % 8 == 0 && !xsum
-        && splitk == 1 && tiles128 >= TR_K32_MIN_TILES)
+        && nz == 1 && tiles128 >= TR_K32_MIN_TILES)
         return launch_tr_ring<false, 32, 3>(a, st);
     constexpr long BN128_MIN_TILES = 384;
     const bool small_n = N <= 64 || tiles128 < BN128_MIN_TILES;
     if (bf16) return small_n ? dispatch_trans<bf16raw, 64>(a, x_trans, w_trans, st) : dispatch_trans<bf16raw, 128>(a, x_trans, w_trans, st);
     return small_n ? dispatch_trans<float, 64>(a, x_trans, w_trans, st) : dispatch_trans<float, 128>(a, x_trans, w_trans, st);
 }
+
+extern "C" int fw_gemm(int dtype, const void* X, long ldx, int x_trans, int x_op, const void* W, long ldw,
+                       int w_trans, int w_op, void* C, long ldc, int out_f32, int accumulate, int M, int N,
+                       int K, float alpha, const float* bias, int act, float slope, const void* aux,
+                       long ldaux, const float* rowscale, int rows_per_scale, const float* residual,
+                       long ldr, int splitk, void* C2, long ldc2, float* xsum, long c_zstride, long xsum_zstride,
+                       void* stream) {
+    return gemm_run(dtype, X, ldx, x_trans, x_op, W, ldw, w_trans, w_op, C, ldc, out_f32, accumulate, M, N, K, alpha, bias, act, slope,
+                    aux, ldaux, rowscale, rows_per_scale, residual, ldr, splitk, C2, ldc2, xsum, c_zstride, xsum_zstride,
+                    nullptr, 0, nullptr, 0, 0, stream);
+}
+
+extern "C" int fw_gemm_splitk(int dtype, const void* X, long ldx, int x_trans, int x_op, const void* W, long ldw,
+                              int w_trans, int w_op, void* C, long ldc, int out_f32, int accumulate, int M, int N,
+                              int K, float alpha, const float* bias, int act, float slope, const void* aux,
+                              long ldaux, const float* rowscale, int rows_per_scale, const float* residual,
+                              long ldr, int splitk, void* C2, long ldc2, float* xsum, long c_zstride, long xsum_zstride,
+                              void* workspace, long workspace_bytes, void* counters, int ncounters, void* stream) {
+    const int rc = gemm_run(dtype, X, ldx, x_trans, x_op, W, ldw, w_trans, w_op, C, ldc, out_f32, accumulate, M, N, K, alpha, bias, act,
+                            slope, aux, ldaux, rowscale, rows_per_scale, residual, ldr, splitk, C2, ldc2, xsum, c_zstride, xsum_zstride,
+                            workspace, workspace_bytes, counters, ncounters, 1, stream);
+    if (rc == 0 && g_auto_sk > 1) {
+        const size_t n = strlen(g_last_kernel);
+        snprintf(g_last_kernel + n, sizeof g_last_kernel - n, "+sk%d", g_auto_sk);
+    }
+    return rc;
+}
diff --git a/frequency-wised_all-in-one_image_restoration_model_amd/fwair/ops.py b/frequency-wised_all-in-one_image_restoration_model_amd/fwair/ops.py
--- a/frequency-wised_all-in-one_image_restoration_model_amd/fwair/ops.py
+++ b/frequency-wised_all-in-one_image_restoration_model_amd/fwair/ops.py
@@ -1,4 +1,5 @@
 import bisect
+import os as _os
 
 import torch
 
@@ -16,7 +17,7 @@
 
 
 def gemm(x, w, M, N, K, *, x_trans=False, w_trans=False, x_op=0, w_op=0, out=None, out_dtype=None, bias=None,
-         act=0, slope=0.0, aux=None, rowscale=None, rows_per_scale=1, residual=None, accumulate=False, splitk=1,
+         act=0, slope=0.0, aux=None, rowscale=None, rows_per_scale=1, residual=None, accumulate=False, splitk=None,
          alpha=1.0, out_gelu=None, xsum=None, c_zstride=0, xsum_zstride=0):
     assert x.dtype == w.dtype
     if out is None:
@@ -26,6 +27,14 @@
     if xsum is not None and not xsum_zstride:
         _note_write(xsum)
     out_f32 = int(out.dtype == torch.float32)
+    if _SPLITK_FUSED and x.dtype == torch.bfloat16 and not (x_trans or accumulate or c_zstride) and xsum is None and splitk != 1:
+        ws, cnt = _splitk_buffers(x.device)
+        call('fw_gemm_splitk', dt(x.dtype), x, _ld(x), 0, x_op, w, _ld(w), int(w_trans), w_op, out, _ld(out), out_f32,
+             0, M, N, K, float(alpha), bias, act, float(slope), aux, _ld(aux) if aux is not None else 0,
+             rowscale, rows_per_scale, residual, _ld(residual) if residual is not None else 0, splitk or 0,
+             out_gelu, _ld(out_gelu) if out_gelu is not None else 0, None, 0, 0, ws, ws.numel(), cnt, cnt.numel())
+        return out
+    splitk = splitk or 1
     call('fw_gemm', dt(x.dtype), x, _ld(x), int(x_trans), x_op, w, _ld(w), int(w_trans), w_op, out, _ld(out), out_f32,
          int(accumulate), M, N, K, float(alpha), bias, act, float(slope), aux, _ld(aux) if aux is not None else 0,
          rowscale, rows_per_scale, residual, _ld(residual) if residual is not None else 0, splitk,
@@ -33,9 +42,24 @@
     return out
 
 
-import os as _os
 _SPLITK_BLOCKS = int(_os.environ.get('FW_SPLITK_BLOCKS', '512'))
 _DGRAD_SPLIT_ROWS = int(_os.environ.get('FW_DGRAD_SPLIT_ROWS', '512'))
+
+
+_SPLITK_FUSED = int(_os.environ.get('FW_SPLITK_FUSED', '1'))
+_SPLITK_WS_BYTES = 32 << 20
+_SPLITK_COUNTERS = 1024
+_SPLITK_MAX = 12
+_splitk_bufs = {}
+
+
+def _splitk_buffers(device):
+    key = (device.index if device.index is not None else torch.cuda.current_device(), torch.cuda.current_stream(device).cuda_stream)
+    bufs = _splitk_bufs.get(key)
+    if bufs is None:
+        bufs = _splitk_bufs[key] = (torch.empty(_SPLITK_WS_BYTES, dtype=torch.uint8, device=device),
+                                    torch.zeros(_SPLITK_COUNTERS, dtype=torch.int32, device=device))
+    return bufs
 
 
 def pick_splitk(M, N, K, dtype):
@@ -342,9 +366,13 @@
 
 def dgrad(g, w, M, K, N, out, act=0, aux=None):
     tiles = ((M + 127) // 128) * ((K + 127) // 128)
-    sk = min(512 // max(tiles, 1), N // _DGRAD_SPLIT_ROWS) if (act == 0 and tiles < 200) else 1
+    fused = bool(_SPLITK_FUSED) and g.dtype == torch.bfloat16
+    sk = min(512 // max(tiles, 1), N // _DGRAD_SPLIT_ROWS) if ((act == 0 or (fused and act == 2)) and tiles < 200) else 1
     if sk <= 1:
         gemm(g, w, M, K, N, w_trans=True, out=out, act=act, aux=aux)
+        return
+    if fused and (sk <= _SPLITK_MAX or act != 0):
+        gemm(g, w, M, K, N, w_trans=True, out=out, act=act, aux=aux, splitk=min(sk, _SPLITK_MAX))
         return
     S = (M * K + 3) // 4 * 4
     slab = torch.empty((sk, S), dtype=torch.float32, device=g.device)
diff --git a/include/fwair.h b/include/fwair.h
--- a/include/fwair.h
+++ b/include/fwair.h
@@ -8,6 +8,11 @@
             void* C, long ldc, int out_f32, int accumulate, int M, int N, int K, float alpha, const float* bias, int act,
             float slope, const void* aux, long ldaux, const float* rowscale, int rows_per_scale, const float* residual,
             long ldr, int splitk, void* C2, long ldc2, float* xsum, long c_zstride, long xsum_zstride, void* stream);
+int fw_gemm_splitk(int dtype, const void* X, long ldx, int x_trans, int x_op, const void* W, long ldw, int w_trans, int w_op,
+                   void* C, long ldc, int out_f32, int accumulate, int M, int N, int K, float alpha, const float* bias, int act,
+                   float slope, const void* aux, long ldaux, const float* rowscale, int rows_per_scale, const float* residual,
+                   long ldr, int splitk, void* C2, long ldc2, float* xsum, long c_zstride, long xsum_zstride, void* workspace,
+                   long workspace_bytes, void* counters, int ncounters, void* stream);
 int fw_gemm_last_kernel(char* buf, int n);
 
 int fw_wgrad_group_prob_bytes(void);
```

Result: no change. 345.0 images/sec, median of 2 (-0.0%).
